# willake/cpu-ray-tracer

Hardware: AMD Instinct MI355X
Metric: Mrays/sec (primary+secondary), 1280x720 64spp path trace — pipelined throughput over 878 consecutive 64-spp windows of one progressive render (single_render = one such render alone) (higher is better)
Workload: dtype f32; 1 GPU; bunny_scene.xml FileScene BVH-SAH path tracer, 1280x720, 64 spp/step (passes=1, depthLimit=5); 1 step = 64 frames = the next spp window of a progressive render; the 878 steps are one crt_render job (14 render kernel launch(es), a wavefront per (tile, 128 consecutive frames), + ordered accumulate), one sync at the end; triangles=4968, parallelism=tile-wave x1

## Files before the change

### cpu-ray-tracer_amd/csrc/abi.cpp

```cpp
#include "../../include/crt_abi.h"
#include "device/launch.h"

#include <cmath>
#include <cstdarg>
#include <cstddef>
#include <cstdio>
#include <cstdlib>
#include <cstring>
#include <deque>
#include <string>
#include <algorithm>
#include <vector>
#include <chrono>

static_assert(sizeof(crt_bvh_node) == 32 && sizeof(crt_tri) == 112 && sizeof(crt_tlas_node) == 32, "reference layouts");
static_assert(sizeof(crt::NodePair) == 64 && sizeof(crt::LeafTri) == 48 && sizeof(crt::ShadeTri) == 64 && sizeof(crt::TlasNode) == 32 &&
              sizeof(crt::Instance) == 128 && sizeof(crt::Material) == 32 && offsetof(crt::Instance, T) == 64, "device layouts");
static_assert(sizeof(crt_counters) == sizeof(crt::Counters), "counter layout");
static_assert(sizeof(crt_kd_node) == 48 && sizeof(crt::KdNode) == sizeof(crt_kd_node) && sizeof(crt::AltTri) == 48, "flat KD node (uploaded as it comes), alternative accelerators' triangle record");
static_assert(offsetof(crt::PrimDev, red) == 536 && sizeof(crt::PrimDev) == 552, "PrimDev: 134 floats, then the two texel pointers");
static_assert(sizeof(crt::BlasAltDesc) == 72, "BLAS descriptor");
static_assert(sizeof(crt_shadow_ray) == 28 && sizeof(crt_ray) == 28 && sizeof(crt_hit) == 28, "query records");
static_assert(sizeof(crt_hit_info) == 48 && offsetof(crt_hit_info, material) == 12 && offsetof(crt_hit_info, N) == 16 && offsetof(crt_hit_info, albedo) == 32 && offsetof(crt_hit_info, v) == 44, "crt_hit_info: three 16-byte pieces");
static_assert(sizeof(crt::Instance) == 128 && offsetof(crt::Instance, triCount) == 112, "Instance record");

namespace {

thread_local std::string g_createError;

bool g_hooks = false;
inline const char* hook(const char* name) { return g_hooks ? getenv(name) : nullptr; }

struct EventPair { hipEvent_t a, b; int mode = -1; bool seen = false; };

}

extern "C" uint32_t crt_debug_query_grid(void)
{
    const char* e = hook("CRT_DEBUG_QUERY_GRID");
    const long k = e ? strtol(e, nullptr, 10) : 0;
    return k > 0 ? (uint32_t)(k > 0x7fffffffL ? 0x7fffffffL : k) : 0u;
}

struct crt_ctx {
    crt_config cfg{};
    std::string err;
    hipStream_t stream = nullptr;
    int tilesX = 0, tilesY = 0;
    uint32_t tileFirst = 0, tileStride = 1, tileCount = 0;
    void* dAccOwned = nullptr; void* dAcc = nullptr;
    std::vector<hipStream_t> streams; uint64_t launchSeq = 0;
    struct Region { size_t off, bytes; hipEvent_t freed; bool held = false; };
    std::deque<Region> inflight;
    char* pool = nullptr; size_t poolBytes = 0, poolHead = 0; bool poolCapped = false;
    hipEvent_t mustWait = nullptr;
    std::vector<hipEvent_t> freeEvents;
    std::vector<hipEvent_t> doneEvents;
    struct Ahead { hipEvent_t end; size_t off; const char* slab; uint64_t epoch; uint32_t sppFirst, nf, passes, used; };
    std::deque<Ahead> ahead;
    uint64_t epoch = 1;
    uint64_t tickEpoch = 0; uint32_t tickNextSpp = 0, tickPasses = 0;
    uint32_t aheadFrames = 0;
    hipStream_t aheadStream = nullptr;
    crt::Scene hScene{};
    crt::Counters* dCounters = nullptr;
    uint32_t* dQueryCursor = nullptr;
    int32_t* dInspectCounts = nullptr; void* dInspectWork = nullptr; size_t inspectCap = 0;
    uint32_t* dPixels = nullptr; float* dTileSums = nullptr;
    unsigned long long* dTileClocks = nullptr;
    std::vector<void*> sceneAllocs;
    float meshLo[3] = {0, 0, 0}, meshHi[3] = {0, 0, 0}; bool orderDirty = true;
    uint32_t* dTileOrder = nullptr;
    uint32_t* hTileOrder[2] = {nullptr, nullptr}; hipEvent_t orderCopied[2] = {nullptr, nullptr}; hipEvent_t orderReady = nullptr; int orderFlip = 0;
    bool haveScene = false;
    struct Flat { int32_t kind = 0; uint64_t leafOff = 0, tlasOff = 0, tlasPairOff = 0, instOff = 0, shadeOff = 0; uint32_t tlasNodeCount = 0, maxHeight = 0;
                  uint32_t objects = 0;
                  std::vector<uint64_t> pairBase, triBase; std::vector<uint32_t> nodesUsed, triCount; std::vector<char> geom;
                  std::vector<float> rootBox; } flat;
    char* hStage[2] = {nullptr, nullptr}; size_t stageBytes[2] = {0, 0}; hipEvent_t stageCopied[2] = {nullptr, nullptr}; int stageFlip = 0;
    hipEvent_t sceneReady = nullptr;
    bool havePrim = false; crt::PrimDev prim{}; uint32_t* dPrimTex = nullptr;
    int renderAccel = 0;
    crt::AltAccelDev alt{}; bool haveKd = false, haveGrid = false; std::vector<void*> altAllocs[2]; crt::AltTri* altTris = nullptr; uint32_t altTriCount = 0;
    crt::TlasAltDev blasAlt[2]{}; bool haveBlas[2] = {false, false}; std::vector<void*> blasAllocs[2];
    bool hasAlt(int kind) const { return (kind == CRT_ACCEL_KDTREE && (haveKd || haveBlas[0])) || (kind == CRT_ACCEL_GRID && (haveGrid || haveBlas[1])); }
    char* dStage = nullptr; size_t stageCap = 0;
    static constexpr int kQuerySlots = 64;
    uint32_t* dQuerySlots = nullptr;
    struct QuerySlot { hipEvent_t done = nullptr; bool pending = false; } qslot[kQuerySlots];
    int qslotNext = 0;
    struct RefitPlan { void* dPlan = nullptr; uint32_t* dLevelOff = nullptr; uint32_t levels = 0, rootCode = 0; bool built = false; };
    std::vector<RefitPlan> refitPlans; std::vector<void*> refitAllocs;
    float* dRefitBack = nullptr; float* hRefitBack = nullptr; hipEvent_t refitFence = nullptr, refitDone = nullptr;
    float* dRootBox = nullptr;
    char* dTlasBuild = nullptr; char* hTlasBack = nullptr; size_t tlasBuildBytes = 0;
    hipEvent_t tlasFence = nullptr, tlasBack = nullptr, tlasDone = nullptr, tlasT0 = nullptr, tlasT1 = nullptr; bool tlasTimed = false;
    hipEvent_t altReady = nullptr;
    static constexpr int kLatStages = 4;
    double tuneMs[kLatStages + 1] = {}; int tuneCount[kLatStages + 1] = {};
    hipEvent_t lastRenderEnd = nullptr;
    int latStage = 0;
    int latBest = 0;
    bool latDone = false;
    bool latConfirming = false; std::vector<int> latQueue;
    bool latWarm = false;
    uint32_t latSlots = 0;
    bool latProbed = false;
    std::vector<uint8_t> latL[kLatStages + 1];
    std::vector<uint32_t> latCost[kLatStages + 1];
    uint32_t* dTileCost = nullptr; uint32_t* hTileCost = nullptr; hipEvent_t costCopied = nullptr; bool costPending = false; int costStage = 0;
    uint32_t* dBlockDesc = nullptr; uint32_t* hBlockDesc = nullptr; uint32_t nBlocks = 0, descCap = 0; hipEvent_t descReady = nullptr;
    uint32_t* dJobCost = nullptr; uint32_t* hJobCost = nullptr; hipEvent_t jobCostCopied = nullptr; bool jobCostPending = false, jobCostValid = false;
    uint32_t recWaves = 0, recResident = 0, recWindows = 0; bool recPool = false;
    double poolWindowTicks = 0;
    std::vector<uint32_t> jobCost;
    std::vector<uint32_t> jobOrder;
    uint32_t* dJobDesc = nullptr; uint32_t* hJobDesc = nullptr; uint32_t jobDescCap = 0, jobBlocks = 0, jobHead = 0; hipEvent_t jobDescReady = nullptr;
    uint32_t planWindows = 0, planFrames = 0; bool planPool = false, planValid = false;
    double jobTrialMs[2] = {0, 0};
    std::vector<hipEvent_t> splitEvents;
    size_t splitSeq = 0; uint32_t splitLaunches = 0;
    uint64_t poolMinWaves = 65000;
    bool usePool = true;
    uint32_t ldsBytes = 0;
    std::vector<EventPair> evPool; size_t evUsedRender = 0, evUsedAcc = 0;
    std::deque<EventPair> evRender, evAcc;
    double foldedRenderMs = 0, foldedAccMs = 0; uint32_t foldedLaunches = 0, poolLaunches = 0;

    int fail(int code, const char* fmt, ...)
    {
        char buf[1024];
        va_list ap; va_start(ap, fmt); vsnprintf(buf, sizeof(buf), fmt, ap); va_end(ap);
        err = buf; return code;
    }
    int hip(hipError_t e, const char* what)
    {
        if (e == hipSuccess) return 0;
        return fail(CRT_ERR_DEVICE, "%s: %s", what, hipGetErrorString(e));
    }
    void freeAlt()
    {
        for (auto& v : altAllocs) { for (void* p : v) (void)hipFree(p); v.clear(); }
        if (altTris) (void)hipFree(altTris);
        altTris = nullptr; altTriCount = 0; haveKd = haveGrid = false; alt = crt::AltAccelDev{}; renderAccel = 0;
        for (int k = 0; k < 2; k++) { for (void* p : blasAllocs[k]) (void)hipFree(p); blasAllocs[k].clear(); haveBlas[k] = false; blasAlt[k] = crt::TlasAltDev{}; }
    }
    void freeScene()
    {
        for (void* p : sceneAllocs) (void)hipFree(p);
        sceneAllocs.clear(); haveScene = false; dRootBox = nullptr;
        for (void* p : refitAllocs) (void)hipFree(p);
        refitAllocs.clear(); refitPlans.clear();
        if (dPrimTex) { (void)hipFree(dPrimTex); dPrimTex = nullptr; }
        havePrim = false;
        freeAlt();
    }
};

#define HIPCK(ctx, call) do { hipError_t e_ = (call); if (e_ != hipSuccess) return (ctx)->hip(e_, #call); } while (0)

namespace {

template <class T>
int upload(crt_ctx* c, const std::vector<T>& v, const T** out)
{
    *out = nullptr;
    if (v.empty()) return 0;
    void* d = nullptr;
    HIPCK(c, hipMalloc(&d, v.size() * sizeof(T)));
    c->sceneAllocs.push_back(d);
    HIPCK(c, hipMemcpyAsync(d, v.data(), v.size() * sizeof(T), hipMemcpyHostToDevice, c->stream));
    HIPCK(c, hipStreamSynchronize(c->stream));
    *out = reinterpret_cast<const T*>(d);
    return 0;
}

template <class T>
int upload_array(crt_ctx* c, std::vector<void*>& allocs, const void* src, size_t bytes, const T** out)
{
    *out = nullptr; if (!bytes) return 0;
    void* d = nullptr; HIPCK(c, hipMalloc(&d, bytes)); allocs.push_back(d);
    HIPCK(c, hipMemcpy(d, src, bytes, hipMemcpyHostToDevice)); *out = static_cast<const T*>(d); return 0;
}

int bvh_height(crt_ctx* c, const crt_bvh& b, uint32_t* heightOut)
{
    std::vector<std::pair<uint32_t, uint32_t>> st; st.push_back({0u, 0u});
    uint32_t h = 0; size_t visited = 0;
    while (!st.empty()) {
        auto [n, d] = st.back(); st.pop_back();
        if (++visited > (size_t)b.nodesUsed) return c->fail(CRT_ERR_INVALID, "BVH node graph is not a tree");
        const crt_bvh_node& nd = b.nodes[n];
        if (nd.triCount > 0) { if (d > h) h = d; continue; }
        if (nd.leftFirst == 0 || nd.leftFirst + 1 >= b.nodesUsed) return c->fail(CRT_ERR_INVALID, "BVH child index out of range (node %u)", n);
        st.push_back({nd.leftFirst, d + 1}); st.push_back({nd.leftFirst + 1, d + 1});
    }
    *heightOut = h;
    return 0;
}

int wait_queries(crt_ctx* c)
{
    for (auto& q : c->qslot) if (q.pending) { HIPCK(c, hipEventSynchronize(q.done)); q.pending = false; }
    return 0;
}

int order_behind_queries(crt_ctx* c)
{
    for (auto& q : c->qslot) {
        if (!q.pending) continue;
        const hipError_t e = hipEventQuery(q.done);
        if (e == hipSuccess) { q.pending = false; continue; }
        if (e != hipErrorNotReady) return c->hip(e, "hipEventQuery(query)");
        HIPCK(c, hipStreamWaitEvent(c->stream, q.done, 0));
    }
    return 0;
}

int drain_all(crt_ctx* c)
{
    for (auto st : c->streams) HIPCK(c, hipStreamSynchronize(st));
    if (c->aheadStream) HIPCK(c, hipStreamSynchronize(c->aheadStream));
    HIPCK(c, hipStreamSynchronize(c->stream));
    return wait_queries(c);
}

}

extern "C" {

int crt_abi_version(void) { return CRT_ABI_VERSION; }

void crt_debug_enable_hooks(int on) { g_hooks = on != 0; }

int crt_device_count(void)
{
    int n = 0;
    if (hipGetDeviceCount(&n) != hipSuccess) return 0;
    return n;
}

const char* crt_last_error(crt_ctx* ctx) { return ctx ? ctx->err.c_str() : g_createError.c_str(); }

int crt_create(crt_ctx** out, const crt_config* cfg)
{
    if (!out || !cfg) { g_createError = "crt_create: null argument"; return CRT_ERR_INVALID; }
    *out = nullptr;
    setenv("GPU_MAX_HW_QUEUES", "16", 0);
    if (cfg->width < 16 || cfg->height < 16) { g_createError = "crt_create: width and height must be at least one 16x16 tile"; return CRT_ERR_INVALID; }
    int ndev = 0;
    hipError_t e = hipGetDeviceCount(&ndev);
    if (e != hipSuccess || ndev == 0) {
        g_createError = "crt_create: no HIP device visible (this library has no CPU path)";
        return CRT_ERR_NO_DEVICE;
    }
    if (cfg->device < 0 || cfg->device >= ndev) { g_createError = "crt_create: device ordinal out of range"; return CRT_ERR_INVALID; }
    crt_ctx* c = new crt_ctx();
    c->cfg = *cfg;
    if (const char* k = hook("CRT_RENDER_KERNEL")) {
        c->usePool = strcmp(k, "tiles") != 0;
        if (!strcmp(k, "pool_always")) c->poolMinWaves = 0;
    }
    if (c->cfg.depthLimit < 0) c->cfg.depthLimit = 5;
    if (c->cfg.depthLimit > 5) { g_createError = "crt_create: depthLimit > 5 unsupported (throughput stack holds 5 factors; reference default is 5)"; delete c; return CRT_ERR_UNSUPPORTED; }
    if (c->cfg.maxFramesPerLaunch <= 0) c->cfg.maxFramesPerLaunch = c->cfg.collectStats ? 64 : 4096;
    if (c->cfg.maxFramesPerLaunch > 64) c->cfg.maxFramesPerLaunch = c->cfg.maxFramesPerLaunch / 64 * 64;
    if (c->cfg.renderStreams < 0) c->cfg.renderStreams = 0;
    c->tilesX = cfg->width / 16; c->tilesY = cfg->height / 16;
    const int tiles = c->tilesX * c->tilesY;
    int first = cfg->tileFirst, stride = cfg->tileStride <= 0 ? 1 : cfg->tileStride, count = cfg->tileCount;
    if (count < 0) { first = 0; stride = 1; count = tiles; }
    if (first < 0 || (count > 0 && (long long)first + (long long)(count - 1) * stride >= tiles)) {
        g_createError = "crt_create: tile range exceeds the image"; delete c; return CRT_ERR_INVALID;
    }
    c->tileFirst = (uint32_t)first; c->tileStride = (uint32_t)stride; c->tileCount = (uint32_t)count;

    auto bail = [&](hipError_t he, const char* what) {
        g_createError = std::string("crt_create: ") + what + ": " + hipGetErrorString(he);
        crt_destroy(c); return CRT_ERR_DEVICE;
    };
    if ((e = hipSetDevice(cfg->device)) != hipSuccess) return bail(e, "hipSetDevice");
    if ((e = hipStreamCreateWithFlags(&c->stream, hipStreamNonBlocking)) != hipSuccess) return bail(e, "hipStreamCreate");
    const size_t px = (size_t)cfg->width * cfg->height;
    if ((e = hipMalloc(&c->dAccOwned, px * 16)) != hipSuccess) return bail(e, "hipMalloc(accumulator)");
    c->dAcc = c->dAccOwned;
    if ((e = hipMemsetAsync(c->dAcc, 0, px * 16, c->stream)) != hipSuccess) return bail(e, "hipMemset(accumulator)");
    if ((e = hipMalloc((void**)&c->dPixels, px * 4)) != hipSuccess) return bail(e, "hipMalloc(pixels)");
    if ((e = hipMemsetAsync(c->dPixels, 0, px * 4, c->stream)) != hipSuccess) return bail(e, "hipMemset(pixels)");
    if ((e = hipMalloc((void**)&c->dTileSums, (size_t)tiles * 4)) != hipSuccess) return bail(e, "hipMalloc(tileSums)");
    if ((e = hipMemsetAsync(c->dTileSums, 0, (size_t)tiles * 4, c->stream)) != hipSuccess) return bail(e, "hipMemset(tileSums)");
    if ((e = hipMalloc((void**)&c->dCounters, sizeof(crt::Counters))) != hipSuccess) return bail(e, "hipMalloc(counters)");
    if ((e = hipMemsetAsync(c->dCounters, 0, sizeof(crt::Counters), c->stream)) != hipSuccess) return bail(e, "hipMemset(counters)");
    if ((e = hipMalloc((void**)&c->dQueryCursor, 64)) != hipSuccess) return bail(e, "hipMalloc(query cursor)");
    if ((e = hipMalloc((void**)&c->dQuerySlots, crt_ctx::kQuerySlots * 64)) != hipSuccess) return bail(e, "hipMalloc(query cursor slots)");
    if (c->cfg.collectStats && count > 0) {
        if ((e = hipMalloc((void**)&c->dTileClocks, (size_t)count * 144)) != hipSuccess) return bail(e, "hipMalloc(tileClocks)");
        if ((e = hipMemsetAsync(c->dTileClocks, 0, (size_t)count * 144, c->stream)) != hipSuccess) return bail(e, "hipMemset(tileClocks)");
    }
    memset(&c->hScene, 0, sizeof(c->hScene));
    const float aspect = (float)cfg->width / (float)cfg->height;
    crt::Scene& s = c->hScene;
    s.camPos[0] = 0; s.camPos[1] = 0; s.camPos[2] = -2;
    s.topLeft[0] = -aspect; s.topLeft[1] = 1; s.topLeft[2] = 0;
    s.topRight[0] = aspect; s.topRight[1] = 1; s.topRight[2] = 0;
    s.bottomLeft[0] = -aspect; s.bottomLeft[1] = -1; s.bottomLeft[2] = 0;
    s.W = cfg->width; s.H = cfg->height; s.invW = 1.0f / cfg->width; s.invH = 1.0f / cfg->height;
    s.depthLimit = c->cfg.depthLimit;
    if ((e = hipStreamSynchronize(c->stream)) != hipSuccess) return bail(e, "hipStreamSynchronize");
    *out = c;
    return CRT_OK;
}

void crt_destroy(crt_ctx* c)
{
    if (!c) return;
    (void)hipSetDevice(c->cfg.device);
    for (auto st : c->streams) (void)hipStreamSynchronize(st);
    if (c->aheadStream) (void)hipStreamSynchronize(c->aheadStream);
    if (c->stream) (void)hipStreamSynchronize(c->stream);
    for (auto& q : c->qslot) if (q.done) { if (q.pending) (void)hipEventSynchronize(q.done); (void)hipEventDestroy(q.done); }
    if (c->dQuerySlots) (void)hipFree(c->dQuerySlots);
    if (c->altReady) (void)hipEventDestroy(c->altReady);
    if (c->refitFence) (void)hipEventDestroy(c->refitFence);
    if (c->refitDone) (void)hipEventDestroy(c->refitDone);
    if (c->dRefitBack) (void)hipFree(c->dRefitBack);
    if (c->hRefitBack) (void)hipHostFree(c->hRefitBack);
    for (hipEvent_t e : {c->tlasFence, c->tlasBack, c->tlasDone, c->tlasT0, c->tlasT1}) if (e) (void)hipEventDestroy(e);
    if (c->dTlasBuild) (void)hipFree(c->dTlasBuild);
    if (c->hTlasBack) (void)hipHostFree(c->hTlasBack);
    c->freeScene();
    for (auto& a : c->ahead) (void)hipEventDestroy(a.end);
    if (c->aheadStream) (void)hipStreamDestroy(c->aheadStream);
    for (auto& ev : c->evPool) { (void)hipEventDestroy(ev.a); (void)hipEventDestroy(ev.b); }
    for (auto& ev : c->evRender) { (void)hipEventDestroy(ev.a); (void)hipEventDestroy(ev.b); }
    for (auto& ev : c->evAcc) { (void)hipEventDestroy(ev.a); (void)hipEventDestroy(ev.b); }
    if (c->dAccOwned) (void)hipFree(c->dAccOwned);
    for (auto st : c->streams) { (void)hipStreamSynchronize(st); (void)hipStreamDestroy(st); }
    for (auto& r : c->inflight) (void)hipEventDestroy(r.freed);
    for (auto e : c->freeEvents) (void)hipEventDestroy(e);
    if (c->mustWait) (void)hipEventDestroy(c->mustWait);
    if (c->pool) (void)hipFree(c->pool);
    for (auto e : c->doneEvents) (void)hipEventDestroy(e);
    if (c->dPixels) (void)hipFree(c->dPixels);
    if (c->dTileSums) (void)hipFree(c->dTileSums);
    if (c->dCounters) (void)hipFree(c->dCounters);
    if (c->dQueryCursor) (void)hipFree(c->dQueryCursor);
    if (c->dInspectCounts) (void)hipFree(c->dInspectCounts);
    if (c->dInspectWork) (void)hipFree(c->dInspectWork);
    if (c->dTileClocks) (void)hipFree(c->dTileClocks);
    if (c->dTileOrder) (void)hipFree(c->dTileOrder);
    if (c->dTileCost) (void)hipFree(c->dTileCost);
    if (c->dJobCost) (void)hipFree(c->dJobCost);
    if (c->dJobDesc) (void)hipFree(c->dJobDesc);
    if (c->hJobDesc) (void)hipHostFree(c->hJobDesc);
    if (c->jobDescReady) (void)hipEventDestroy(c->jobDescReady);
    if (c->hJobCost) (void)hipHostFree(c->hJobCost);
    if (c->jobCostCopied) (void)hipEventDestroy(c->jobCostCopied);
    for (auto e : c->splitEvents) (void)hipEventDestroy(e);
    if (c->hTileCost) (void)hipHostFree(c->hTileCost);
    if (c->costCopied) (void)hipEventDestroy(c->costCopied);
    if (c->dBlockDesc) (void)hipFree(c->dBlockDesc);
    if (c->hBlockDesc) (void)hipHostFree(c->hBlockDesc);
    if (c->descReady) (void)hipEventDestroy(c->descReady);
    if (c->dStage) (void)hipFree(c->dStage);
    for (int k = 0; k < 2; k++) { if (c->hTileOrder[k]) (void)hipHostFree(c->hTileOrder[k]); if (c->orderCopied[k]) (void)hipEventDestroy(c->orderCopied[k]); }
    for (int k = 0; k < 2; k++) { if (c->hStage[k]) (void)hipHostFree(c->hStage[k]); if (c->stageCopied[k]) (void)hipEventDestroy(c->stageCopied[k]); }
    if (c->stream) (void)hipStreamDestroy(c->stream);
    delete c;
}

int crt_upload_scene(crt_ctx* c, const crt_scene_desc* sd)
{
    if (!c || !sd) return CRT_ERR_INVALID;
    c->epoch++;
    HIPCK(c, hipSetDevice(c->cfg.device));
    if (sd->kind != CRT_SCENE_FILE && sd->kind != CRT_SCENE_TLAS) return c->fail(CRT_ERR_INVALID, "unknown scene kind %d", sd->kind);
    if (!sd->bvhs || sd->bvhCount == 0) return c->fail(CRT_ERR_INVALID, "scene has no acceleration structure");
    if (sd->kind == CRT_SCENE_FILE && sd->bvhCount != 1) return c->fail(CRT_ERR_INVALID, "CRT_SCENE_FILE takes exactly one BVH (FileScene::acc)");
    if (sd->kind == CRT_SCENE_TLAS && (sd->bvhCount > 256 || !sd->tlasNodes || sd->tlasNodeCount < 2 * sd->bvhCount))
        return c->fail(CRT_ERR_INVALID, "TLAS scene needs <= 256 BLAS (tlas_bvh.cpp:21) and 2*blasCount TLAS nodes");
    if (sd->textureCount == 0 || !sd->textures) return c->fail(CRT_ERR_INVALID, "floor and skydome textures are required");
    if (sd->floorTexture < 0 || sd->floorTexture >= (int)sd->textureCount || sd->skyTexture < 0 || sd->skyTexture >= (int)sd->textureCount)
        return c->fail(CRT_ERR_INVALID, "floor/sky texture index out of range");
    for (uint32_t i = 0; i < sd->textureCount; i++)
        if (!sd->textures[i].pixels || sd->textures[i].width <= 0 || sd->textures[i].height <= 0) return c->fail(CRT_ERR_INVALID, "texture %u is empty", i);
    if (sd->materialCount > 0 && !sd->materials) return c->fail(CRT_ERR_INVALID, "materialCount is %u but materials is NULL", sd->materialCount);
    for (uint32_t i = 0; i < sd->materialCount; i++)
        if (sd->materials[i].texture >= (int)sd->textureCount) return c->fail(CRT_ERR_INVALID, "material %u: texture index out of range", i);
    if (sd->kind == CRT_SCENE_FILE) {
        if (!sd->objMatIdx || sd->objCount == 0) return c->fail(CRT_ERR_INVALID, "CRT_SCENE_FILE needs objMatIdx");
        for (uint32_t i = 0; i < sd->objCount; i++)
            if (sd->objMatIdx[i] < 0 || sd->objMatIdx[i] >= (int)sd->materialCount) return c->fail(CRT_ERR_INVALID, "objMatIdx entry out of range");
    }

    uint64_t nPairs = 0, nTris = 0;
    uint32_t maxHeight = 0;
    for (uint32_t bi = 0; bi < sd->bvhCount; bi++) {
        const crt_bvh& b = sd->bvhs[bi];
        if (!b.nodes || !b.triangles || !b.triangleIndices || b.nodesUsed == 0 || b.triCount == 0) return c->fail(CRT_ERR_INVALID, "BVH %u is empty", bi);
        if ((b.nodesUsed & 1u) == 0) return c->fail(CRT_ERR_INVALID, "BVH %u: nodesUsed must be odd (root + child pairs)", bi);
        if (sd->kind == CRT_SCENE_TLAS && (b.matIdx < 0 || b.matIdx >= (int)sd->materialCount)) return c->fail(CRT_ERR_INVALID, "BLAS %u: matIdx out of range", bi);
        if (sd->kind == CRT_SCENE_TLAS && b.objIdx != (int)bi + 2)
            return c->fail(CRT_ERR_INVALID, "BLAS %u: objIdx must be %u (TLASFileScene numbers objects from 2, tlas_file_scene.cpp:13,51-53)", bi, bi + 2);
        uint32_t h = 0; int r = bvh_height(c, b, &h); if (r) return r;
        if (h > maxHeight) maxHeight = h;
        nPairs += b.nodesUsed / 2; nTris += b.triCount;
    }
    const uint64_t pairBytes = nPairs ? nPairs * 64 : 64;
    const uint64_t leafOffB = pairBytes, leafBytes = (nTris + 1) * 48;
    const uint64_t tlasOffB = (leafOffB + leafBytes + 63) & ~63ull;
    const uint64_t tlasBytes = (sd->kind == CRT_SCENE_TLAS) ? (uint64_t)sd->tlasNodeCount * 32 : 0;
    const uint64_t tlasPairOffB = (tlasOffB + tlasBytes + 63) & ~63ull;
    const uint64_t tlasPairBytes = (sd->kind == CRT_SCENE_TLAS) ? (uint64_t)sd->tlasNodeCount * 32 : 0;
    const uint64_t instOffB = (tlasPairOffB + tlasPairBytes + 127) & ~127ull;
    const uint64_t instBytes = (sd->kind == CRT_SCENE_TLAS) ? (uint64_t)sd->bvhCount * 128 : 0;
    const uint64_t shadeOffB = (instOffB + instBytes + 63) & ~63ull;
    const uint64_t total = shadeOffB + nTris * 64;
    if (total >= crt::kMaxGeomBytes) return c->fail(CRT_ERR_UNSUPPORTED, "scene geometry needs %llu bytes; this build addresses 4 GiB", (unsigned long long)total);
    if (sd->kind == CRT_SCENE_TLAS && sd->tlasNodeCount > 0x7fffu) return c->fail(CRT_ERR_UNSUPPORTED, "TLAS node index exceeds 15 bits");

    std::vector<char> geom((size_t)total, 0);
    crt::NodePair* pairs = reinterpret_cast<crt::NodePair*>(geom.data());
// ... 475 lines not shown
    for (uint32_t i = 0; i < n; i++) if (lanes[i] == 0 || lanes[i] > 64 || (64 % lanes[i]) != 0) return CRT_ERR_INVALID;
    std::vector<uint8_t> L; const double t = solve_block_table(std::vector<uint8_t>(lanes, lanes + n), std::vector<uint32_t>(cost, cost + n), budget, L);
    if (n) memcpy(out, L.data(), n);
    if (T) *T = t;
    return CRT_OK;
}
static double lat_budget(crt_ctx* c)
{
    if (!c->latSlots) c->latSlots = crt_render_resident_waves(c->cfg.device, c->hScene.kind, c->ldsBytes);
    double share = 0.98;
    if (const char* e = hook("CRT_LAT_BUDGET")) { const double v = atof(e); if (v > 0) share = v; }
    return share * (double)c->latSlots;
}

static int upload_block_table(crt_ctx* c, const std::vector<uint8_t>& lanes, const std::vector<uint32_t>& cost)
{
    const uint32_t n = c->tileCount;
    std::vector<uint32_t> order(n);
    for (uint32_t i = 0; i < n; i++) order[i] = i;
    std::stable_sort(order.begin(), order.end(), [&](uint32_t a, uint32_t b) { return cost[a] > cost[b]; });
    std::vector<uint32_t> table; table.reserve((size_t)n * 2);
    for (uint32_t r = 0; r < n; r++) {
        const uint32_t tl = order[r], L = lanes[tl];
        for (uint32_t base = 0; base < 64u; base += L) table.push_back(block_desc(tl, base, L, 0u));
    }
    if (table.size() > 0x7fffffffull) return c->fail(CRT_ERR_INVALID, "block table too large");
    if (hook("CRT_LAT_VERBOSE")) fprintf(stderr, "[crt] latency table: %zu wavefronts for %u tiles (slowest tile of the base stage %.2f ms)\n", table.size(), n, n ? cost[order[0]] * 1e-5 : 0.0);
    if (c->descCap < table.size()) {
        if (c->dBlockDesc) (void)hipFree(c->dBlockDesc);
        if (c->hBlockDesc) (void)hipHostFree(c->hBlockDesc);
        c->dBlockDesc = nullptr; c->hBlockDesc = nullptr; c->descCap = 0;
        const size_t cap = table.size() + table.size() / 2;
        HIPCK(c, hipMalloc((void**)&c->dBlockDesc, cap * 4));
        HIPCK(c, hipHostMalloc((void**)&c->hBlockDesc, cap * 4, hipHostMallocDefault));
        c->descCap = (uint32_t)cap;
    } else if (c->descReady) HIPCK(c, hipEventSynchronize(c->descReady));
    if (!c->descReady) HIPCK(c, hipEventCreateWithFlags(&c->descReady, hipEventDisableTiming));
    memcpy(c->hBlockDesc, table.data(), table.size() * 4);
    { const int r = order_behind_ahead(c); if (r) return r; }
    HIPCK(c, hipMemcpyAsync(c->dBlockDesc, c->hBlockDesc, table.size() * 4, hipMemcpyHostToDevice, c->stream));
    HIPCK(c, hipEventRecord(c->descReady, c->stream));
    c->nBlocks = (uint32_t)table.size();
    return 0;
}

static int next_block_table(crt_ctx* c)
{
    const uint32_t n = c->tileCount; const int K = crt_ctx::kLatStages;
    const int s = c->costStage;
    if (s == 0 && !c->latWarm && !c->latProbed) { c->latWarm = true; return 0; }
    c->latCost[s].assign(c->hTileCost, c->hTileCost + n);
    if (s == 0 && !c->latProbed) c->latL[0].assign(n, 64);
    if (c->tuneCount[s] && (c->latBest == s || !c->tuneCount[c->latBest] || c->tuneMs[s] < c->tuneMs[c->latBest])) c->latBest = s;
    bool last = s >= K;
    std::vector<std::pair<double, uint32_t>> steps;
    if (const char* e = hook("CRT_LAT_POLICY")) {
        for (const char* p = e; *p;) {
            char* q = nullptr; const double sh = strtod(p, &q); if (q == p || *q != ':') break;
            const long L = strtol(q + 1, &q, 10); if (L < 1 || L > 64 || (64 % L) != 0) break;
            steps.push_back({sh, (uint32_t)L});
            p = (*q == ',') ? q + 1 : q; if (*q != ',') break;
        }
        if (s >= 1) last = true;
    }
    auto install = [&](int stage) -> int {
        if ((stage != 0 || c->latProbed) && stage != c->latStage) { const int r = upload_block_table(c, c->latL[stage], c->latCost[stage]); if (r) return r; }
        c->latStage = stage; return 0;
    };
    auto fastest = [&](int except) { int b = -1; for (int k = 0; k <= K; k++) if (k != except && c->tuneCount[k] && (b < 0 || c->tuneMs[k] < c->tuneMs[b])) b = k; return b; };
    auto finish = [&]() -> int {
        c->latDone = true; c->latConfirming = false;
        const int b = fastest(-1); c->latBest = b < 0 ? 0 : b;
        if (hook("CRT_LAT_FORCE")) c->latBest = s;
        if (hook("CRT_LAT_VERBOSE")) { fprintf(stderr, "[crt] latency stages:"); for (int k = 0; k <= K; k++) if (c->tuneCount[k]) fprintf(stderr, " %d: %.2f ms", k, c->tuneMs[k]); fprintf(stderr, " -> %d\n", c->latBest); }
        return install(c->latBest);
    };
    if (c->latConfirming) {
        if (!c->latQueue.empty()) c->latQueue.erase(c->latQueue.begin());
        if (!c->latQueue.empty()) return install(c->latQueue.front());
        return finish();
    }
    if (last) {
        const int a = fastest(-1), b2 = fastest(a);
        if (hook("CRT_LAT_FORCE") || a < 0 || b2 < 0) return finish();
        c->latQueue = {a, b2}; c->latConfirming = true;
        return install(a);
    }
    const int b = c->latBest;
    const std::vector<uint8_t>& baseL = c->latL[b]; const std::vector<uint32_t>& baseC = c->latCost[b];
    uint32_t top = 0; for (uint32_t i = 0; i < n; i++) top = baseC[i] > top ? baseC[i] : top;
    std::vector<uint8_t>& L = c->latL[s + 1]; L = baseL;
    if (!steps.empty()) {
        for (uint32_t i = 0; i < n; i++)
            for (const auto& st : steps) if (top > 0 && (double)baseC[i] >= st.first * (double)top) { L[i] = (uint8_t)st.second; break; }
    } else {
        const double T = solve_block_table(c->latL[s], c->latCost[s], lat_budget(c), L);
        if (hook("CRT_LAT_VERBOSE")) fprintf(stderr, "[crt] stage %d: aim %.2f ms\n", s + 1, T * 1e-5);
    }
    const int r = upload_block_table(c, L, steps.empty() ? c->latCost[s] : baseC);
    if (r) return r;
    c->latStage = s + 1;
    return 0;
}

static void harvest_tuning(crt_ctx* c)
{
    for (auto& ev : c->evRender) {
        if (ev.mode < 0 || ev.seen) continue;
        if (hipEventQuery(ev.b) != hipSuccess) break;
        float t = 0;
        if (hipEventElapsedTime(&t, ev.a, ev.b) == hipSuccess) {
            if (ev.mode >= 100) { double& m = c->jobTrialMs[ev.mode - 100]; m = (m > 0 && m < t) ? m : t; }
            else { c->tuneMs[ev.mode] = c->tuneCount[ev.mode] ? (c->tuneMs[ev.mode] < t ? c->tuneMs[ev.mode] : t) : t; c->tuneCount[ev.mode]++; }
        }
        ev.seen = true;
    }
}

static void fold_completed(crt_ctx* c, std::deque<EventPair>& list, double* ms, uint32_t* count)
{
    while (list.size() > 64 && hipEventQuery(list.front().b) == hipSuccess) {
        float t = 0;
        if (hipEventElapsedTime(&t, list.front().a, list.front().b) == hipSuccess) *ms += t;
        if (count) (*count)++;
        c->evPool.push_back(list.front()); list.pop_front();
    }
}

static int take_event(crt_ctx* c, std::deque<EventPair>& list, EventPair* out)
{
    EventPair ev;
    if (c->evPool.empty()) {
        HIPCK(c, hipEventCreate(&ev.a)); HIPCK(c, hipEventCreate(&ev.b));
    } else { ev = c->evPool.back(); c->evPool.pop_back(); }
    ev.mode = -1; ev.seen = false;
    list.push_back(ev); *out = ev;
    return 0;
}

static int release_ahead_region(crt_ctx* c, const crt_ctx::Ahead& a)
{
    for (auto& r : c->inflight)
        if (r.held && r.off == a.off) { HIPCK(c, hipEventRecord(r.freed, c->stream)); r.held = false; return 0; }
    return c->fail(CRT_ERR_DEVICE, "render-ahead region at %zu is not in the slab ring", a.off);
}

static int discard_ahead(crt_ctx* c)
{
    while (!c->ahead.empty()) {
        const crt_ctx::Ahead a = c->ahead.front(); c->ahead.pop_front();
        HIPCK(c, hipStreamWaitEvent(c->stream, a.end, 0));
        c->doneEvents.push_back(a.end);
        const int r = release_ahead_region(c, a); if (r) return r;
    }
    c->aheadFrames = 0;
    return 0;
}

static int ensure_pool(crt_ctx* c, uint32_t frames, uint32_t passes, uint32_t* maxFOut)
{
    const size_t windowBytes = window_bytes(c, passes);
    uint32_t maxF = (uint32_t)c->cfg.maxFramesPerLaunch;
    uint32_t maxW = maxF >= 64u ? maxF / 64u : 1u;
    const uint32_t wantW = (frames + 63u) / 64u;
    const uint32_t callW = wantW < maxW ? wantW : maxW;
    size_t want = (size_t)callW * windowBytes * (wantW > callW ? 2u : 1u);
    if (want < 8 * windowBytes) want = 8 * windowBytes;
    if (want > c->poolBytes && !(c->poolCapped && windowBytes <= c->poolBytes)) {
        { const int r = discard_ahead(c); if (r) return r; }
        HIPCK(c, hipStreamSynchronize(c->stream));
        for (auto st : c->streams) HIPCK(c, hipStreamSynchronize(st));
        if (c->aheadStream) HIPCK(c, hipStreamSynchronize(c->aheadStream));
        for (auto& r : c->inflight) c->freeEvents.push_back(r.freed);
        c->inflight.clear(); c->poolHead = 0;
        if (c->pool) { HIPCK(c, hipFree(c->pool)); c->pool = nullptr; c->poolBytes = 0; }
        size_t freeB = 0, totalB = 0;
        HIPCK(c, hipMemGetInfo(&freeB, &totalB));
        const size_t budget = freeB / 2;
        if (budget < windowBytes) return c->fail(CRT_ERR_DEVICE, "not enough free HBM for one 64-frame sample slab (%zu bytes needed, %zu free)", windowBytes, freeB);
        c->poolCapped = want > budget;
        if (want > budget) want = budget;
        want = want / windowBytes * windowBytes;
        HIPCK(c, hipMalloc((void**)&c->pool, want));
        c->poolBytes = want;
    }
    {
        uint32_t fitW = (uint32_t)(c->poolBytes / windowBytes);
        if (wantW > fitW && fitW >= 2) fitW /= 2;
        if (maxW > fitW) maxW = fitW;
    }
    if (maxF >= 64u) maxF = maxW * 64u;
    *maxFOut = maxF;
    return 0;
}

int crt_reserve(crt_ctx* c, uint32_t frames, uint32_t passes)
{
    if (!c) return CRT_ERR_INVALID;
    if (passes < 1 || passes > 4) return c->fail(CRT_ERR_INVALID, "passes must be 1..4");
    HIPCK(c, hipSetDevice(c->cfg.device));
    { const int r = discard_ahead(c); if (r) return r; }
    if (c->tileCount == 0 || frames == 0) return CRT_OK;
    uint32_t maxF = 0;
    return ensure_pool(c, frames, passes, &maxF);
}

static int take_region(crt_ctx* c, size_t need, hipStream_t st, size_t* offOut)
{
    for (;;) {
        bool ok = false; size_t off = 0;
        if (c->inflight.empty()) { off = 0; ok = need <= c->poolBytes; }
        else {
            const size_t tail = c->inflight.front().off;
            if (c->poolHead > tail) {
                if (c->poolBytes - c->poolHead >= need) { off = c->poolHead; ok = true; }
                else if (tail >= need) { off = 0; ok = true; }
            } else if (c->poolHead < tail && tail - c->poolHead >= need) { off = c->poolHead; ok = true; }
        }
        if (ok) {
            if (c->mustWait) HIPCK(c, hipStreamWaitEvent(st, c->mustWait, 0));
            c->poolHead = off + need; *offOut = off;
            return 0;
        }
        if (c->inflight.empty()) return c->fail(CRT_ERR_DEVICE, "slab pool of %zu bytes cannot hold a launch of %zu bytes", c->poolBytes, need);
        if (c->inflight.front().held) return 1;
        if (c->mustWait) c->freeEvents.push_back(c->mustWait);
        c->mustWait = c->inflight.front().freed;
        c->inflight.pop_front();
    }
}

static size_t job_cost_clk_offset(const crt_ctx* c) { return (((size_t)c->tileCount + 1u) & ~(size_t)1u) * 4u; }
static size_t job_cost_bytes(const crt_ctx* c) { return job_cost_clk_offset(c) + 24u; }

static int adopt_job_costs(crt_ctx* c)
{
    const uint32_t n = c->tileCount;
    c->jobCost.assign(c->hJobCost, c->hJobCost + n);
    {
        const unsigned long long* clk = reinterpret_cast<const unsigned long long*>(reinterpret_cast<const char*>(c->hJobCost) + job_cost_clk_offset(c));
        const double s0 = (clk[0] && clk[1] && clk[1] > ~clk[0]) ? (double)(clk[1] - ~clk[0]) : 0.0;
        const double drain = (double)clk[2] / (double)(c->recResident ? c->recResident : 1u);
        c->poolWindowTicks = 0;
        if (c->recWindows && (double)c->recWaves >= 1.5 * (double)c->recResident && s0 > 0) c->poolWindowTicks = (s0 + drain) / (double)c->recWindows / (c->recPool ? 1.0 : 1.2);
        if (hook("CRT_LAT_VERBOSE")) fprintf(stderr, "[crt] measured %u windows with %s: %u wavefronts, last one started %.2f ms after the first, then %.2f ms of drain -> %.3f ms of machine time per window under the pool\n", c->recWindows, c->recPool ? "the pool" : "one stream per lane", c->recWaves, s0 * 1e-5, drain * 1e-5, c->poolWindowTicks * 1e-5);
    }
    c->jobOrder.resize(n);
    for (uint32_t i = 0; i < n; i++) c->jobOrder[i] = i;
    std::stable_sort(c->jobOrder.begin(), c->jobOrder.end(), [&](uint32_t a, uint32_t b) { return c->jobCost[a] > c->jobCost[b]; });
    c->jobCostValid = true; c->planValid = false;
    return upload_tile_order(c, c->jobOrder);
}

static void plan_job(const crt_ctx* c, uint32_t windows, uint32_t frames, bool pool, std::vector<uint32_t>& table, uint32_t* head)
{
    table.clear(); *head = 0;
    const uint32_t n = c->tileCount;
    if (!c->jobCostValid || windows < 2u || windows > 64u || n > 0x10000u || c->cfg.collectStats || hook("CRT_SPLIT_OFF")) return;
    if (pool && c->streams.size() < 2) return;
    if (const char* e = hook("CRT_SPLIT_FORCE")) {
        const uint32_t h = std::min<uint32_t>((uint32_t)atoi(e), pool ? n - 1u : n);
        static const uint32_t Ls[4] = {64u, 16u, 2u, 1u};
        for (uint32_t r = 0; r < (pool ? h : n); r++) { const uint32_t L = r < h ? Ls[r & 3u] : 64u; for (uint32_t w = 0; w < windows; w++) for (uint32_t b0 = 0; b0 < 64u; b0 += L) table.push_back(block_desc(c->jobOrder[r], b0, L, w)); }
        *head = h; return;
    }
    double poolLong = 2.4, wideLoad = 1.1, poolSlots = 4096.0, wideMt = 1.2, narrowSlots = 3500.0;
    if (const char* e = hook("CRT_PLAN_NARROW_SLOTS")) narrowSlots = atof(e);
    const double K = (double)windows;
    double costSum = 0; for (uint32_t v : c->jobCost) costSum += (double)v;
    const double perCost = (c->poolWindowTicks > 0 && costSum > 0) ? c->poolWindowTicks / costSum : 1.0 / poolSlots;
    auto cheapest = [&](double v, double T, int* cls) -> double {
        if (pool && poolLong * v <= T) { *cls = 0; return K * v * perCost; }
        if (wideLoad * v <= T) { *cls = 1; return K * wideMt * v * perCost; }
        int k = 1; while (k < 6 && kLatG[k] * v > T) k++;
        *cls = 2 + k; return K * (64.0 / kLatLanes[k]) * kLatG[k] * v / narrowSlots;
    };
    auto machine = [&](double T) { double m = 0; int cls; for (uint32_t v : c->jobCost) m += cheapest((double)v, T, &cls); return m; };
    const double top = (double)c->jobCost[c->jobOrder[0]];
    double lo = top * kLatG[6], hi = std::max(poolLong * top, machine(1e30)) * 1.01;
    if (machine(lo) <= lo) hi = lo;
    else for (int it = 0; it < 50; it++) { const double mid = 0.5 * (lo + hi); if (machine(mid) <= mid) hi = mid; else lo = mid; }
    const double T = hi;
    uint32_t h = 0, narrow = 0; std::vector<uint8_t> lanes(n, 64);
    for (uint32_t r = 0; r < n; r++) {
        int cls; (void)cheapest((double)c->jobCost[c->jobOrder[r]], T, &cls);
        if (cls != 0) h = r + 1u;
        if (cls >= 2) { lanes[r] = (uint8_t)kLatLanes[cls - 2]; narrow++; }
    }
    if (pool && h >= n) h = n - 1u;
    if (hook("CRT_LAT_VERBOSE")) fprintf(stderr, "[crt] job of %u windows, %u tiles: makespan aim %.1f ms (most expensive tile %.2f ms); %u tiles to the block table, %u of them narrow, %s\n", windows, n, T * 1e-5, top * 1e-5, pool ? h : (narrow ? n : 0u), narrow, pool ? "rest to the pool" : "no pool");
    if (pool ? h == 0u : narrow == 0u) return;
    const uint32_t upto = pool ? h : n;
    for (uint32_t r = 0; r < upto; r++) {
        const uint32_t L = lanes[r];
        for (uint32_t w = 0; w < windows; w++) {
            const uint32_t fw = std::min(64u, frames - w * 64u);
            for (uint32_t b0 = 0; b0 < fw; b0 += L) table.push_back(block_desc(c->jobOrder[r], b0, L, w));
        }
    }
    if (table.size() > (4u << 20)) { table.clear(); *head = 0; return; }
    *head = pool ? h : 0u;
}

static int install_job_plan(crt_ctx* c, uint32_t windows, uint32_t frames, bool pool)
{
    if (c->planValid && c->planWindows == windows && c->planFrames == frames && c->planPool == pool) return 0;
    std::vector<uint32_t> table; uint32_t head = 0;
    plan_job(c, windows, frames, pool, table, &head);
    c->planValid = true; c->planWindows = windows; c->planFrames = frames; c->planPool = pool; c->jobHead = head; c->jobBlocks = (uint32_t)table.size();
    c->jobTrialMs[0] = c->jobTrialMs[1] = 0;
    if (table.empty()) return 0;
    if (c->jobDescCap < table.size()) {
        if (c->dJobDesc) (void)hipFree(c->dJobDesc);
        if (c->hJobDesc) (void)hipHostFree(c->hJobDesc);
        c->dJobDesc = nullptr; c->hJobDesc = nullptr; c->jobDescCap = 0;
        const size_t cap = table.size() + table.size() / 2;
        HIPCK(c, hipMalloc((void**)&c->dJobDesc, cap * 4));
        HIPCK(c, hipHostMalloc((void**)&c->hJobDesc, cap * 4, hipHostMallocDefault));
        c->jobDescCap = (uint32_t)cap;
    } else if (c->jobDescReady) HIPCK(c, hipEventSynchronize(c->jobDescReady));
    if (!c->jobDescReady) HIPCK(c, hipEventCreateWithFlags(&c->jobDescReady, hipEventDisableTiming));
    memcpy(c->hJobDesc, table.data(), table.size() * 4);
    { const int r = order_behind_ahead(c); if (r) return r; }
    HIPCK(c, hipMemcpyAsync(c->dJobDesc, c->hJobDesc, table.size() * 4, hipMemcpyHostToDevice, c->stream));
    HIPCK(c, hipEventRecord(c->jobDescReady, c->stream));
    return 0;
}

struct Launch {
    hipStream_t st = nullptr; EventPair ev{}; void* slab = nullptr; uint32_t sppFirst = 0, nf = 0, passes = 1, windows = 1;
    const uint32_t* blockDesc = nullptr; uint32_t nBlocks = 0;
    bool wantCost = false, wantJobCost = false, pool = false;
    uint32_t head = 0, jobBlocks = 0; unsigned long long* jobClk = nullptr;
};

static int next_block_table(crt_ctx* c);
static int probe_tile_costs(crt_ctx* c, hipStream_t st);

static int tuner_prepare(crt_ctx* c, Launch& L)
{
    int r;
    const bool gpuIdle = !c->lastRenderEnd || hipEventQuery(c->lastRenderEnd) == hipSuccess;
    if (L.nf <= 64u && L.nf >= 8u && gpuIdle && !c->cfg.collectStats && c->tileCount <= 0x10000u && !hook("CRT_LAT_OFF")) {
        if (c->costPending && hipEventQuery(c->costCopied) == hipSuccess) { c->costPending = false; harvest_tuning(c); if ((r = next_block_table(c))) return r; }
        if (c->latStage == 0 && !c->latProbed && !c->latWarm && !c->costPending && L.nf == 64u && !hook("CRT_LAT_POLICY") && !hook("CRT_LAT_NO_PROBE")) { if ((r = probe_tile_costs(c, L.st))) return r; }
        const int stage = c->latStage;
        if (stage || c->latProbed) { L.blockDesc = c->dBlockDesc; L.nBlocks = c->nBlocks; HIPCK(c, hipStreamWaitEvent(L.st, c->descReady, 0)); }
        L.wantCost = (!c->latDone && !c->costPending) || (c->latDone && hook("CRT_LAT_RECORD"));
        c->evRender.back().mode = c->latDone ? -1 : stage;
        if (L.wantCost && !c->latDone) c->costStage = stage;
    }
    if (L.wantCost) {
        if (!c->dTileCost) {
            HIPCK(c, hipMalloc((void**)&c->dTileCost, (size_t)c->tileCount * 4));
            HIPCK(c, hipHostMalloc((void**)&c->hTileCost, (size_t)c->tileCount * 4, hipHostMallocDefault));
            HIPCK(c, hipEventCreateWithFlags(&c->costCopied, hipEventDisableTiming));
        }
        else HIPCK(c, hipStreamWaitEvent(L.st, c->costCopied, 0));
        HIPCK(c, hipMemsetAsync(c->dTileCost, 0, (size_t)c->tileCount * 4, L.st));
    }
    return 0;
}

static int planner_prepare(crt_ctx* c, Launch& L)
{
    int r;
    if (L.nf > 64u && !c->cfg.collectStats) {
        if (c->jobCostPending && hipEventQuery(c->jobCostCopied) == hipSuccess) { c->jobCostPending = false; if ((r = adopt_job_costs(c))) return r; HIPCK(c, hipStreamWaitEvent(L.st, c->orderReady, 0)); }
        L.wantJobCost = !c->jobCostValid && !c->jobCostPending && L.nf >= 128u;
        if (L.wantJobCost) {
            if (!c->dJobCost) {
                HIPCK(c, hipMalloc((void**)&c->dJobCost, job_cost_bytes(c)));
                HIPCK(c, hipHostMalloc((void**)&c->hJobCost, job_cost_bytes(c), hipHostMallocDefault));
                HIPCK(c, hipEventCreateWithFlags(&c->jobCostCopied, hipEventDisableTiming));
            } else HIPCK(c, hipStreamWaitEvent(L.st, c->jobCostCopied, 0));
            HIPCK(c, hipMemsetAsync(c->dJobCost, 0, job_cost_bytes(c), L.st));
        }
    }
    const uint64_t minWaves = c->poolMinWaves != 65000u ? c->poolMinWaves : (c->jobCostValid ? 43000u : 65000u);
    L.pool = c->usePool && c->hScene.ref16ok && (uint64_t)c->tileCount * L.windows >= minWaves && (c->poolMinWaves == 0 || L.nf > 64u);
    if (L.nf > 64u && c->jobCostValid) {
        if ((r = install_job_plan(c, L.windows, L.nf, L.pool))) return r;
        int use = 1;
        if (c->jobBlocks && !hook("CRT_PLAN_NO_TRIAL")) {
            if (c->jobTrialMs[1] > 0 && c->jobTrialMs[0] > 0) use = c->jobTrialMs[1] <= c->jobTrialMs[0] ? 1 : 0;
            else if (c->jobTrialMs[1] > 0 && c->jobTrialMs[0] == 0) use = 0;
            c->evRender.back().mode = 100 + use;
        }
        if (use) { L.head = c->jobHead; L.jobBlocks = c->jobBlocks; }
    }
    if (L.jobBlocks) HIPCK(c, hipStreamWaitEvent(L.st, c->jobDescReady, 0));
    if (L.wantJobCost) {
        L.jobClk = reinterpret_cast<unsigned long long*>(reinterpret_cast<char*>(c->dJobCost) + job_cost_clk_offset(c));
        c->recPool = L.pool; c->recWindows = L.windows;
        c->recWaves = L.pool ? c->tileCount * ((L.nf + crt_pool_streams(L.nf) - 1u) / crt_pool_streams(L.nf)) : c->tileCount * L.windows;
        c->recResident = L.pool ? 4096u : 5120u;
    }
    return 0;
}

static hipError_t launch_render_kernels(crt_ctx* c, const Launch& L)
{
    hipStream_t st = L.st;
    hipError_t le = hipSuccess;
    auto join = [&](hipStream_t other) -> hipError_t {
        if (other == st) return hipSuccess;
        hipError_t e = hipSuccess;
        if (c->splitEvents.size() < 32) { hipEvent_t ne; e = hipEventCreateWithFlags(&ne, hipEventDisableTiming); if (e == hipSuccess) c->splitEvents.push_back(ne); }
        if (e == hipSuccess) { hipEvent_t je = c->splitEvents[c->splitSeq++ % c->splitEvents.size()]; e = hipEventRecord(je, other); if (e == hipSuccess) e = hipStreamWaitEvent(st, je, 0); }
        return e;
    };
    auto launch_table = [&](const uint32_t* desc, uint32_t nBlocks, uint32_t* cost) -> hipError_t {
        return crt_launch_render(&c->hScene, L.slab, c->dCounters, c->dTileClocks, c->dTileOrder, c->tileFirst, c->tileStride, c->tileCount, (uint32_t)c->tilesX,
                                 L.sppFirst, L.nf, L.passes, c->ldsBytes, 0, desc, nBlocks, cost, 0u, nullptr, st);
    };
    if (L.pool) {
        void* scratch = (char*)L.slab + (size_t)L.windows * sample_bytes_per_window(c, L.passes);
        hipStream_t st2 = st;
        if (L.jobBlocks) {
            le = launch_table(c->dJobDesc, L.jobBlocks, nullptr);
            st2 = c->streams[(size_t)(c->launchSeq++ % c->streams.size())];
            if (le == hipSuccess && st2 != st) le = hipStreamWaitEvent(st2, L.ev.a, 0);
        }
        if (le == hipSuccess)
            le = crt_launch_render_pool(&c->hScene, L.slab, scratch, c->dCounters, c->dTileClocks, c->dTileOrder, c->tileFirst, c->tileStride, c->tileCount, (uint32_t)c->tilesX,
                                        L.sppFirst, L.nf, L.passes, c->cfg.collectStats, L.jobBlocks ? L.head : 0u, L.wantJobCost ? c->dJobCost : nullptr, L.jobClk, st2);
        if (L.jobBlocks && le == hipSuccess) le = join(st2);
    } else if (L.jobBlocks) {
        le = launch_table(c->dJobDesc, L.jobBlocks, nullptr);
    } else if (L.blockDesc && L.nBlocks) {
        le = launch_table(L.blockDesc, L.nBlocks, L.wantCost ? c->dTileCost : nullptr);
    } else {
        le = crt_launch_render(&c->hScene, L.slab, c->dCounters, c->dTileClocks, c->dTileOrder, c->tileFirst, c->tileStride, c->tileCount, (uint32_t)c->tilesX,
                               L.sppFirst, L.nf, L.passes, c->ldsBytes, c->cfg.collectStats, nullptr, 0u,
                               L.wantCost ? c->dTileCost : (L.wantJobCost ? c->dJobCost : nullptr), 0u, L.jobClk, st);
    }
    if (L.jobBlocks && le == hipSuccess) c->splitLaunches++;
    return le;
}

static int probe_tile_costs(crt_ctx* c, hipStream_t st)
{
    const uint32_t n = c->tileCount;
    if (!c->dTileCost) {
        HIPCK(c, hipMalloc((void**)&c->dTileCost, (size_t)n * 4));
        HIPCK(c, hipHostMalloc((void**)&c->hTileCost, (size_t)n * 4, hipHostMallocDefault));
        HIPCK(c, hipEventCreateWithFlags(&c->costCopied, hipEventDisableTiming));
    } else HIPCK(c, hipEventSynchronize(c->costCopied));
    const auto tp0 = std::chrono::steady_clock::now();
    HIPCK(c, crt_launch_probe(&c->hScene, c->tileFirst, c->tileStride, n, (uint32_t)c->tilesX, c->dTileCost, st));
    HIPCK(c, hipMemcpyAsync(c->hTileCost, c->dTileCost, (size_t)n * 4, hipMemcpyDeviceToHost, st));
    HIPCK(c, hipEventRecord(c->costCopied, st));
    HIPCK(c, hipStreamSynchronize(st));
    const auto tp1 = std::chrono::steady_clock::now();
    std::vector<uint32_t>& est = c->latCost[0]; est.assign(c->hTileCost, c->hTileCost + n);
    for (uint32_t i = 0; i < n; i++) est[i] += 18u * crt_probe_paths();
    std::vector<uint8_t>& L = c->latL[0]; L.assign(n, 64);
    solve_block_table(std::vector<uint8_t>(n, 64), est, lat_budget(c), L);
    c->latProbed = true;
    bool any = false; for (uint32_t i = 0; i < n; i++) any = any || L[i] != 64;
    if (!any) { c->latProbed = false; return 0; }
    const auto tp2 = std::chrono::steady_clock::now();
    const int r = upload_block_table(c, L, est);
    if (hook("CRT_LAT_VERBOSE")) { const auto tp3 = std::chrono::steady_clock::now(); auto ms = [](auto a, auto b) { return std::chrono::duration<double, std::milli>(b - a).count(); };
        fprintf(stderr, "[crt] cost probe: launch + wait %.3f ms, table solved in %.3f ms, uploaded in %.3f ms\n", ms(tp0, tp1), ms(tp1, tp2), ms(tp2, tp3)); }
    return r;
}

static int launch_frames(crt_ctx* c, uint32_t sppFirst, uint32_t nf, uint32_t passes, hipStream_t st, crt_ctx::Ahead* ahead)
{
    const size_t windowBytes = window_bytes(c, passes);
    size_t off = 0; int r;
    if ((r = take_region(c, (size_t)((nf + 63u) / 64u) * windowBytes, st, &off))) return r;
    if (c->orderReady) HIPCK(c, hipStreamWaitEvent(st, c->orderReady, 0));
    if (c->sceneReady) HIPCK(c, hipStreamWaitEvent(st, c->sceneReady, 0));
    void* slab = c->pool + off;
    EventPair ev;
    harvest_tuning(c);
    fold_completed(c, c->evRender, &c->foldedRenderMs, &c->foldedLaunches); fold_completed(c, c->evAcc, &c->foldedAccMs, nullptr);
    if ((r = take_event(c, c->evRender, &ev))) return r;
    struct PairGuard { crt_ctx* c; bool armed; ~PairGuard() { if (armed && !c->evRender.empty()) { c->evPool.push_back(c->evRender.back()); c->evRender.pop_back(); } } } pairGuard{c, true};
    Launch L; L.st = st; L.ev = ev; L.slab = slab; L.sppFirst = sppFirst; L.nf = nf; L.passes = passes; L.windows = (nf + 63u) / 64u;
    if ((r = tuner_prepare(c, L))) return r;
    if ((r = planner_prepare(c, L))) return r;
    HIPCK(c, hipEventRecord(ev.a, st));
    const bool pool = L.pool, wantCost = L.wantCost, wantJobCost = L.wantJobCost;
    const hipError_t le = hook("CRT_DEBUG_FAIL_LAUNCH") ? hipErrorInvalidConfiguration  : launch_render_kernels(c, L);
    if (le != hipSuccess) {
        return c->hip(le, pool ? "launch of render_pool_kernel" : "launch of render_tiles_kernel");
    }
    if (pool) c->poolLaunches++;
    HIPCK(c, hipEventRecord(ev.b, st));
    pairGuard.armed = false;
    c->lastRenderEnd = ev.b;
    if (wantJobCost) {
        HIPCK(c, hipMemcpyAsync(c->hJobCost, c->dJobCost, job_cost_bytes(c), hipMemcpyDeviceToHost, st));
        HIPCK(c, hipEventRecord(c->jobCostCopied, st));
        c->jobCostPending = true;
    }
    if (wantCost && !pool && !c->latDone) {
        HIPCK(c, hipMemcpyAsync(c->hTileCost, c->dTileCost, (size_t)c->tileCount * 4, hipMemcpyDeviceToHost, st));
        HIPCK(c, hipEventRecord(c->costCopied, st));
        c->costPending = true;
    }
    crt_ctx::Region reg; reg.off = off; reg.bytes = (size_t)((nf + 63u) / 64u) * windowBytes;
    if (c->freeEvents.empty()) HIPCK(c, hipEventCreateWithFlags(&reg.freed, hipEventDisableTiming));
    else { reg.freed = c->freeEvents.back(); c->freeEvents.pop_back(); }
    if (ahead) {
        hipEvent_t end = nullptr;
        if (c->doneEvents.empty()) { const hipError_t e = hipEventCreateWithFlags(&end, hipEventDisableTiming); if (e != hipSuccess) { c->freeEvents.push_back(reg.freed); return c->hip(e, "hipEventCreate"); } }
        else { end = c->doneEvents.back(); c->doneEvents.pop_back(); }
        const hipError_t e = hipEventRecord(end, st);
        if (e != hipSuccess) { c->doneEvents.push_back(end); c->freeEvents.push_back(reg.freed); return c->hip(e, "hipEventRecord"); }
        reg.held = true;
        c->inflight.push_back(reg);
        *ahead = crt_ctx::Ahead{end, off, (const char*)slab, c->epoch, sppFirst, nf, passes, 0u};
        return 0;
    }
    HIPCK(c, hipStreamWaitEvent(c->stream, ev.b, 0));
    if ((r = take_event(c, c->evAcc, &ev))) return r;
    HIPCK(c, hipEventRecord(ev.a, c->stream));
    HIPCK(c, crt_launch_accumulate(slab, c->dAcc, c->tileFirst, c->tileStride, c->tileCount, (uint32_t)c->tilesX, (uint32_t)c->cfg.width, nf, passes, c->stream));
    HIPCK(c, hipEventRecord(ev.b, c->stream));
    HIPCK(c, hipEventRecord(reg.freed, c->stream));
    c->inflight.push_back(reg);
    return 0;
}

int crt_render(crt_ctx* c, uint32_t spp_first, uint32_t frames, uint32_t passes)
{
    if (!c) return CRT_ERR_INVALID;
    if (!c->haveScene && !c->havePrim) return c->fail(CRT_ERR_STATE, "crt_render before crt_upload_scene");
    if (passes < 1 || passes > 4) return c->fail(CRT_ERR_INVALID, "passes must be 1..4 (the reference's UI range, renderer.cpp:178)");
    HIPCK(c, hipSetDevice(c->cfg.device));
    { int r = discard_ahead(c); if (r) return r; }
    if (c->tileCount == 0 || frames == 0) return CRT_OK;
    { int r = update_tile_order(c); if (r) return r; }
    if (c->streams.empty()) {
        int n = c->cfg.renderStreams;
        if (n <= 0) n = 7;
        if (n > 16) n = 16;
        if (c->cfg.collectStats) n = 1;
        c->streams.resize((size_t)n);
        for (auto& st : c->streams) HIPCK(c, hipStreamCreateWithFlags(&st, hipStreamNonBlocking));
    }
    uint32_t maxF = 0;
    { int r = ensure_pool(c, frames, passes, &maxF); if (r) return r; }
    const size_t windowBytes = window_bytes(c, passes);
    if (c->renderAccel != 0 || c->havePrim) {
        for (uint32_t f0 = 0; f0 < frames; f0 += maxF) {
            const uint32_t nf = (frames - f0 < maxF) ? frames - f0 : maxF;
            size_t off = 0; int r;
            if ((r = take_region(c, (size_t)((nf + 63u) / 64u) * windowBytes, c->stream, &off))) return r;
            if (c->sceneReady) HIPCK(c, hipStreamWaitEvent(c->stream, c->sceneReady, 0));
            void* slab = c->pool + off;
            if (c->havePrim) HIPCK(c, crt_launch_render_prim(&c->hScene, &c->prim, slab, c->dCounters, c->tileFirst, c->tileStride, c->tileCount, (uint32_t)c->tilesX, spp_first + f0 * passes, nf, passes, c->stream));
            else HIPCK(c, crt_launch_render_alt(c->renderAccel, &c->hScene, &c->alt, &c->blasAlt[c->renderAccel - 1], slab, c->dCounters, c->tileFirst, c->tileStride, c->tileCount, (uint32_t)c->tilesX, spp_first + f0 * passes, nf, passes, c->stream));
            HIPCK(c, crt_launch_accumulate(slab, c->dAcc, c->tileFirst, c->tileStride, c->tileCount, (uint32_t)c->tilesX, (uint32_t)c->cfg.width, nf, passes, c->stream));
            crt_ctx::Region reg; reg.off = off; reg.bytes = (size_t)((nf + 63u) / 64u) * windowBytes;
            if (c->freeEvents.empty()) HIPCK(c, hipEventCreateWithFlags(&reg.freed, hipEventDisableTiming));
            else { reg.freed = c->freeEvents.back(); c->freeEvents.pop_back(); }
            HIPCK(c, hipEventRecord(reg.freed, c->stream));
            c->inflight.push_back(reg);
        }
        return CRT_OK;
    }
    for (uint32_t f0 = 0; f0 < frames; f0 += maxF) {
        const uint32_t nf = (frames - f0 < maxF) ? frames - f0 : maxF;
        const int r = launch_frames(c, spp_first + f0 * passes, nf, passes, c->streams[(size_t)(c->launchSeq++ % c->streams.size())], nullptr);
        if (r) return r > 0 ? c->fail(CRT_ERR_DEVICE, "slab ring blocked by a render-ahead region") : r;
    }
    return CRT_OK;
}

int crt_sync(crt_ctx* c)
{
    if (!c) return CRT_ERR_INVALID;
    HIPCK(c, hipSetDevice(c->cfg.device));
    HIPCK(c, hipStreamSynchronize(c->stream));
    for (auto st : c->streams) HIPCK(c, hipStreamSynchronize(st));
    if (c->aheadStream) HIPCK(c, hipStreamSynchronize(c->aheadStream));
    return CRT_OK;
}

int crt_clear(crt_ctx* c)
{
    if (!c) return CRT_ERR_INVALID;
    HIPCK(c, hipSetDevice(c->cfg.device));
    HIPCK(c, hipMemsetAsync(c->dAcc, 0, (size_t)c->cfg.width * c->cfg.height * 16, c->stream));
    return CRT_OK;
}

int crt_read_accumulator(crt_ctx* c, float* host)
{
    if (!c || !host) return CRT_ERR_INVALID;
    HIPCK(c, hipSetDevice(c->cfg.device));
    HIPCK(c, hipMemcpyAsync(host, c->dAcc, (size_t)c->cfg.width * c->cfg.height * 16, hipMemcpyDeviceToHost, c->stream));
    HIPCK(c, hipStreamSynchronize(c->stream));
    return CRT_OK;
}

static int read_screen(crt_ctx* c, uint32_t* hostPixels, float* energy)
{
    const int tiles = c->tilesX * c->tilesY;
    if (hostPixels) HIPCK(c, hipMemcpyAsync(hostPixels, c->dPixels, (size_t)c->cfg.width * c->cfg.height * 4, hipMemcpyDeviceToHost, c->stream));
    std::vector<float> sums(tiles);
    HIPCK(c, hipMemcpyAsync(sums.data(), c->dTileSums, (size_t)tiles * 4, hipMemcpyDeviceToHost, c->stream));
    HIPCK(c, hipStreamSynchronize(c->stream));
    if (energy) { float e = 0; for (int i = 0; i < tiles; i++) e += sums[i]; *energy = e; }
    return CRT_OK;
}

int crt_resolve_screen(crt_ctx* c, float scale, uint32_t* hostPixels, float* energy)
{
    if (!c) return CRT_ERR_INVALID;
    HIPCK(c, hipSetDevice(c->cfg.device));
    HIPCK(c, crt_launch_resolve(c->dAcc, c->dPixels, c->dTileSums, c->tileFirst, c->tileStride, c->tileCount, (uint32_t)c->tilesX, (uint32_t)c->cfg.width, scale, c->stream));
    return read_screen(c, hostPixels, energy);
}

static constexpr uint32_t kAheadMaxFrames = 256;

static int launch_ahead(crt_ctx* c, uint32_t sppFirst, uint32_t passes)
{
    if (!c->aheadStream) {
        int least = 0, greatest = 0;
        HIPCK(c, hipDeviceGetStreamPriorityRange(&least, &greatest));
        HIPCK(c, hipStreamCreateWithPriority(&c->aheadStream, hipStreamNonBlocking, least));
    }
    uint32_t nf = c->aheadFrames ? std::min(2u * c->aheadFrames, kAheadMaxFrames) : 64u;
    if (nf > (uint32_t)c->cfg.maxFramesPerLaunch) nf = (uint32_t)c->cfg.maxFramesPerLaunch;
    const uint32_t poolW = (uint32_t)(c->poolBytes / window_bytes(c, passes));
    if (nf > poolW / 2u * 64u) nf = poolW / 2u * 64u;
    if (nf == 0 || c->streams.empty()) return 0;
    hipStream_t st = hook("CRT_AHEAD_NORMAL_PRIORITY") ? c->streams[(size_t)(c->launchSeq++ % c->streams.size())] : c->aheadStream;
    crt_ctx::Ahead a{};
    const int r = launch_frames(c, sppFirst, nf, passes, st, &a);
    if (r < 0) return r;
    if (r > 0) return 0;
    c->ahead.push_back(a); c->aheadFrames = nf;
    return 0;
}

int crt_tick(crt_ctx* c, uint32_t spp, uint32_t passes, uint32_t* hostPixels, float* hostRgba, float* energy)
{
    if (!c) return CRT_ERR_INVALID;
    if (!c->haveScene && !c->havePrim) return c->fail(CRT_ERR_STATE, "crt_tick before crt_upload_scene");
    if (passes < 1 || passes > 4) return c->fail(CRT_ERR_INVALID, "passes must be 1..4 (the reference's UI range, renderer.cpp:178)");
    HIPCK(c, hipSetDevice(c->cfg.device));
    const float scale = 1.0f / (float)(spp + passes);
    const bool eligible = !c->cfg.collectStats && c->renderAccel == 0 && !c->havePrim && c->tileCount > 0;
    const bool streak = eligible && c->tickEpoch == c->epoch && spp == c->tickNextSpp && passes == c->tickPasses;
    c->tickEpoch = c->epoch; c->tickNextSpp = spp + passes; c->tickPasses = passes;
    const bool hit = !c->ahead.empty() && c->ahead.front().epoch == c->epoch && c->ahead.front().passes == passes &&
                     spp == c->ahead.front().sppFirst + c->ahead.front().used * passes;
    int r;
    if (hit) {
        crt_ctx::Ahead& a = c->ahead.front();
        const uint32_t f = a.used++;
        HIPCK(c, hipStreamWaitEvent(c->stream, a.end, 0));
        HIPCK(c, crt_launch_commit_frame(a.slab + (size_t)(f / 64u) * sample_bytes_per_window(c, passes), f % 64u, passes, c->dAcc, c->dPixels, c->dTileSums,
                                         c->tileFirst, c->tileStride, c->tileCount, (uint32_t)c->tilesX, (uint32_t)c->cfg.width, scale, c->stream));
        if (a.used == a.nf) {
            const crt_ctx::Ahead done = a; c->ahead.pop_front();
            c->doneEvents.push_back(done.end);
            if ((r = release_ahead_region(c, done))) return r;
        }
        if (c->ahead.size() < 2u) {
            const uint32_t next = c->ahead.empty() ? spp + passes : c->ahead.back().sppFirst + c->ahead.back().nf * passes;
            if ((r = launch_ahead(c, next, passes))) return r;
        }
    } else {
        if ((r = crt_render(c, spp, 1, passes))) return r;
        HIPCK(c, crt_launch_resolve(c->dAcc, c->dPixels, c->dTileSums, c->tileFirst, c->tileStride, c->tileCount, (uint32_t)c->tilesX, (uint32_t)c->cfg.width, scale, c->stream));
    }
    if (hostRgba) HIPCK(c, hipMemcpyAsync(hostRgba, c->dAcc, (size_t)c->cfg.width * c->cfg.height * 16, hipMemcpyDeviceToHost, c->stream));
    if ((r = read_screen(c, hostPixels, energy))) return r;
    if (!hit && streak && (r = launch_ahead(c, spp + passes, passes))) return r;
    return CRT_OK;
}

int crt_whitted_tick(crt_ctx* c, uint32_t* hostPixels)
{
    if (!c) return CRT_ERR_INVALID;
    if (!c->haveScene) return c->fail(CRT_ERR_STATE, "crt_whitted_tick before crt_upload_scene");
    HIPCK(c, hipSetDevice(c->cfg.device));
    HIPCK(c, crt_launch_whitted(&c->hScene, c->renderAccel, &c->alt, c->renderAccel ? &c->blasAlt[c->renderAccel - 1] : nullptr, c->dAcc, c->dPixels, c->dCounters, c->ldsBytes, c->stream));
    if (hostPixels) HIPCK(c, hipMemcpyAsync(hostPixels, c->dPixels, (size_t)c->cfg.width * c->cfg.height * 4, hipMemcpyDeviceToHost, c->stream));
    HIPCK(c, hipStreamSynchronize(c->stream));
    return CRT_OK;
}

int crt_whitted_tick_inspect(crt_ctx* c, int inspect, int32_t peakTraversalIn, int32_t peakTestsIn, uint32_t* hostPixels, int32_t* hostTraversed, int32_t* hostTested, crt_whitted_metrics* metrics)
{
    if (!c) return CRT_ERR_INVALID;
    if (inspect < CRT_INSPECT_NONE || inspect > CRT_INSPECT_TESTS) return c->fail(CRT_ERR_INVALID, "crt_whitted_tick_inspect: inspect must be CRT_INSPECT_NONE, _TRAVERSAL or _TESTS");
    if (peakTraversalIn < 0 || peakTestsIn < 0) return c->fail(CRT_ERR_INVALID, "crt_whitted_tick_inspect: a peak cannot be negative");
    if (!c->haveScene) return c->fail(CRT_ERR_STATE, "crt_whitted_tick_inspect before crt_upload_scene");
    HIPCK(c, hipSetDevice(c->cfg.device));
    const size_t n = (size_t)c->cfg.width * c->cfg.height;
    if (n > c->inspectCap) {
        HIPCK(c, hipStreamSynchronize(c->stream));
        if (c->dInspectCounts) (void)hipFree(c->dInspectCounts);
        if (c->dInspectWork) (void)hipFree(c->dInspectWork);
        c->dInspectCounts = nullptr; c->dInspectWork = nullptr; c->inspectCap = 0;
        HIPCK(c, hipMalloc((void**)&c->dInspectCounts, n * 2 * sizeof(int32_t)));
        HIPCK(c, hipMalloc(&c->dInspectWork, crt_whitted_inspect_work_bytes((uint32_t)n)));
        c->inspectCap = n;
    }
    int32_t* dTrav = c->dInspectCounts; int32_t* dTested = c->dInspectCounts + n;
    HIPCK(c, crt_launch_whitted_inspect(&c->hScene, c->renderAccel, &c->alt, c->renderAccel ? &c->blasAlt[c->renderAccel - 1] : nullptr, inspect,
                                        inspect == CRT_INSPECT_TESTS ? peakTestsIn : peakTraversalIn, c->dAcc, c->dPixels, c->dCounters, dTrav, dTested, c->dInspectWork, c->ldsBytes, c->stream));
    static_assert(sizeof(crt_whitted_metrics) == 32, "crt::InspectSums (kernels.hip) is read back into this record");
    crt_whitted_metrics m;
    if (hostPixels) HIPCK(c, hipMemcpyAsync(hostPixels, c->dPixels, n * 4, hipMemcpyDeviceToHost, c->stream));
    if (hostTraversed) HIPCK(c, hipMemcpyAsync(hostTraversed, dTrav, n * 4, hipMemcpyDeviceToHost, c->stream));
    if (hostTested) HIPCK(c, hipMemcpyAsync(hostTested, dTested, n * 4, hipMemcpyDeviceToHost, c->stream));
    if (metrics) HIPCK(c, hipMemcpyAsync(&m, c->dInspectWork, sizeof(m), hipMemcpyDeviceToHost, c->stream));
    HIPCK(c, hipStreamSynchronize(c->stream));
    if (metrics) {
        if (m.peakTraversal < peakTraversalIn) m.peakTraversal = peakTraversalIn;
        if (m.peakTests < peakTestsIn) m.peakTests = peakTestsIn;
        *metrics = m;
    }
    return CRT_OK;
}

static int stage(crt_ctx* c, size_t bytes)
{
// ... 484 lines not shown
        HIPCK(c, hipStreamWaitEvent(st, c->tlasFence, 0));
    }
    HIPCK(c, hipMemcpyAsync(const_cast<char*>(c->hScene.geom) + f.tlasOff, c->dTlasBuild + sizeof(crt::TlasBuildHeader), imageBytes, hipMemcpyDeviceToDevice, st));
    HIPCK(c, hipEventRecord(c->tlasDone, st));
    c->sceneReady = c->tlasDone;
    if (st != c->stream) HIPCK(c, hipStreamWaitEvent(c->stream, c->tlasDone, 0));
    c->epoch++;
    memcpy(f.geom.data() + f.tlasOff, image, imageBytes);
    const crt::TlasNode* nodes = reinterpret_cast<const crt::TlasNode*>(image);
    adopt_tlas(c, h.height, nodes[0].lo, nodes[0].hi);
    if (tlasOut)
        for (uint32_t i = 0; i < 2u * N; i++) {
            const crt::TlasNode& n = nodes[i]; crt_tlas_node& o = tlasOut[i];
            memcpy(o.aabbMin, n.lo, 12); memcpy(o.aabbMax, n.hi, 12);
            const bool leaf = (n.ref & 0xC0000000u) == crt::kRefTlasLeaf;
            o.leftRight = leaf ? 0u : ((n.ref & 0x7fffu) | (((n.ref >> 15) & 0x7fffu) << 16));
            o.BLAS = leaf ? (n.ref & 0xffffu) : 0u;
        }
    return CRT_OK;
}

extern "C" int crt_internal_read_device(crt_ctx* c, void* dst, const void* d_src, size_t bytes, void* stream)
{
    if (!c || !dst) return CRT_ERR_INVALID;
    HIPCK(c, hipSetDevice(c->cfg.device));
    int r; hipStream_t st = nullptr;
    if ((r = check_device_buffer(c, d_src, bytes, "crt_internal_read_device")) || (r = caller_stream(c, stream, "crt_internal_read_device", &st))) return r;
    HIPCK(c, hipMemcpyAsync(dst, d_src, bytes, hipMemcpyDeviceToHost, st));
    HIPCK(c, hipStreamSynchronize(st));
    return CRT_OK;
}

extern "C" int crt_debug_tlas_build_ms(crt_ctx* c, float* ms)
{
    if (!c || !ms) return CRT_ERR_INVALID;
    if (!c->tlasTimed) return c->fail(CRT_ERR_STATE, "crt_debug_tlas_build_ms: no timed crt_update_transforms_device (debug hooks off?)");
    HIPCK(c, hipEventSynchronize(c->tlasT1));
    HIPCK(c, hipEventElapsedTime(ms, c->tlasT0, c->tlasT1));
    return CRT_OK;
}

int crt_is_occluded(crt_ctx* c, int accel, const crt_shadow_ray* rays, int32_t* occluded, size_t n)
{
    if (!c) return CRT_ERR_INVALID;
    int r;
    if ((r = query_check(c, accel, true, n, "crt_is_occluded"))) return r;
    if (n == 0) return CRT_OK;
    if (!rays || !occluded) return c->fail(CRT_ERR_INVALID, "crt_is_occluded: NULL buffer");
    return query_host(c, true, accel, rays, occluded, n);
}

static int shade_check(crt_ctx* c, bool hitInfo, size_t n, const char* what)
{
    if (hitInfo && c->havePrim) return c->fail(CRT_ERR_UNSUPPORTED, "%s: GetHitInfo of the PrimitiveScene is not served (crt_abi.h)", what);
    return query_check(c, 0, false, n, what);
}

static uint32_t file_tri_count(const crt_ctx* c) { return c->flat.kind == CRT_SCENE_FILE ? c->flat.triCount[0] : 0u; }

int crt_get_hit_info(crt_ctx* c, const crt_ray* rays, const crt_hit* hits, crt_hit_info* out, size_t n)
{
    if (!c) return CRT_ERR_INVALID;
    int r;
    if ((r = shade_check(c, true, n, "crt_get_hit_info"))) return r;
    if (n == 0) return CRT_OK;
    if (!rays || !hits || !out) return c->fail(CRT_ERR_INVALID, "crt_get_hit_info: NULL buffer");
    const crt_ctx::Flat& f = c->flat;
    for (size_t i = 0; i < n; i++)
        if (!crt::hit_record_ok(hits[i].objIdx, hits[i].triIdx, f.objects, [&](uint32_t k) { return f.triCount[f.kind == CRT_SCENE_TLAS ? k : 0]; }))
            return c->fail(CRT_ERR_INVALID, "crt_get_hit_info: record %zu names objIdx %d, triIdx %d; the scene has objects -1 .. %u and that object's BVH fewer triangles", i, hits[i].objIdx, hits[i].triIdx, f.objects + 1);
    HIPCK(c, hipSetDevice(c->cfg.device));
    if ((r = stage(c, n * (sizeof(crt_hit_info) + sizeof(crt_ray) + sizeof(crt_hit))))) return r;
    char* dOut = c->dStage; char* dRays = dOut + n * sizeof(crt_hit_info); char* dHits = dRays + n * sizeof(crt_ray);
    HIPCK(c, hipMemcpyAsync(dRays, rays, n * sizeof(crt_ray), hipMemcpyHostToDevice, c->stream));
    HIPCK(c, hipMemcpyAsync(dHits, hits, n * sizeof(crt_hit), hipMemcpyHostToDevice, c->stream));
    HIPCK(c, crt_launch_hit_info(&c->hScene, dRays, dHits, dOut, (uint32_t)n, f.objects, file_tri_count(c), c->stream));
    HIPCK(c, hipMemcpyAsync(out, dOut, n * sizeof(crt_hit_info), hipMemcpyDeviceToHost, c->stream));
    HIPCK(c, hipStreamSynchronize(c->stream));
    return CRT_OK;
}

int crt_get_hit_info_device(crt_ctx* c, const crt_ray* d_rays, const crt_hit* d_hits, crt_hit_info* d_out, size_t n, void* stream)
{
    if (!c) return CRT_ERR_INVALID;
    const char* what = "crt_get_hit_info_device";
    int r;
    if ((r = shade_check(c, true, n, what))) return r;
    if (n == 0) return CRT_OK;
    HIPCK(c, hipSetDevice(c->cfg.device));
    if ((r = check_device_buffer(c, d_rays, n * sizeof(crt_ray), what)) || (r = check_device_buffer(c, d_hits, n * sizeof(crt_hit), what)) ||
        (r = check_device_buffer(c, d_out, n * sizeof(crt_hit_info), what))) return r;
    if (reinterpret_cast<uintptr_t>(d_out) & 15u) return c->fail(CRT_ERR_INVALID, "%s: the output buffer %p is not 16-byte aligned", what, (void*)d_out);
    hipStream_t st = nullptr; int k = 0;
    if ((r = begin_device_query(c, stream, what, &st, &k))) return r;
    HIPCK(c, crt_launch_hit_info(&c->hScene, d_rays, d_hits, d_out, (uint32_t)n, c->flat.objects, file_tri_count(c), st));
    return end_device_query(c, k, st);
}

int crt_get_sky_color(crt_ctx* c, const crt_ray* rays, float* rgb, size_t n)
{
    if (!c) return CRT_ERR_INVALID;
    int r;
    if ((r = shade_check(c, false, n, "crt_get_sky_color"))) return r;
    if (n == 0) return CRT_OK;
    if (!rays || !rgb) return c->fail(CRT_ERR_INVALID, "crt_get_sky_color: NULL buffer");
    if (c->havePrim) { memset(rgb, 0, n * 12); return CRT_OK; }
    HIPCK(c, hipSetDevice(c->cfg.device));
    if ((r = stage(c, n * (12 + sizeof(crt_ray))))) return r;
    float* dOut = reinterpret_cast<float*>(c->dStage); char* dRays = c->dStage + n * 12;
    HIPCK(c, hipMemcpyAsync(dRays, rays, n * sizeof(crt_ray), hipMemcpyHostToDevice, c->stream));
    HIPCK(c, crt_launch_sky_color(&c->hScene, dRays, dOut, (uint32_t)n, c->stream));
    HIPCK(c, hipMemcpyAsync(rgb, dOut, n * 12, hipMemcpyDeviceToHost, c->stream));
    HIPCK(c, hipStreamSynchronize(c->stream));
    return CRT_OK;
}

int crt_get_sky_color_device(crt_ctx* c, const crt_ray* d_rays, float* d_rgb, size_t n, void* stream)
{
    if (!c) return CRT_ERR_INVALID;
    const char* what = "crt_get_sky_color_device";
    int r;
    if ((r = shade_check(c, false, n, what))) return r;
    if (n == 0) return CRT_OK;
    HIPCK(c, hipSetDevice(c->cfg.device));
    if ((r = check_device_buffer(c, d_rays, n * sizeof(crt_ray), what)) || (r = check_device_buffer(c, d_rgb, n * 12, what))) return r;
    hipStream_t st = nullptr; int k = 0;
    if ((r = begin_device_query(c, stream, what, &st, &k))) return r;
    if (c->havePrim) HIPCK(c, hipMemsetAsync(d_rgb, 0, n * 12, st));
    else HIPCK(c, crt_launch_sky_color(&c->hScene, d_rays, d_rgb, (uint32_t)n, st));
    return end_device_query(c, k, st);
}

static int sample_check(crt_ctx* c, int accel, size_t n, const char* what)
{
    int r;
    if ((r = query_check(c, accel, false, n, what))) return r;
    const uint32_t words = sample_stack_words(c, accel);
    if (!sample_lds_fits(words)) return c->fail(CRT_ERR_UNSUPPORTED, "%s: a traversal stack of %u dwords per lane exceeds the kernel's LDS", what, words);
    return 0;
}

static hipError_t launch_sample(crt_ctx* c, int accel, const void* rays, uint32_t* seeds, float* rgb, uint32_t n, uint32_t* cursor, uint32_t* residentLanes, hipStream_t st)
{
    if (c->havePrim) return crt_launch_sample_query_prim(&c->hScene, &c->prim, rays, seeds, rgb, n, c->dCounters, cursor, residentLanes, st);
    return crt_launch_sample_query(accel, &c->hScene, &c->alt, accel ? &c->blasAlt[accel - 1] : nullptr, rays, seeds, rgb, n, c->dCounters, cursor, residentLanes, st);
}

int crt_sample(crt_ctx* c, int accel, const crt_ray* rays, uint32_t* seeds, float* rgb, size_t n)
{
    if (!c) return CRT_ERR_INVALID;
    int r;
    if ((r = sample_check(c, accel, n, "crt_sample"))) return r;
    if (n == 0) return CRT_OK;
    if (!rays || !seeds || !rgb) return c->fail(CRT_ERR_INVALID, "crt_sample: NULL buffer");
    HIPCK(c, hipSetDevice(c->cfg.device));
    if ((r = stage(c, n * (12 + sizeof(crt_ray) + 4)))) return r;
    float* dRgb = reinterpret_cast<float*>(c->dStage); char* dRays = c->dStage + n * 12; uint32_t* dSeeds = reinterpret_cast<uint32_t*>(dRays + n * sizeof(crt_ray));
    HIPCK(c, hipMemcpyAsync(dRays, rays, n * sizeof(crt_ray), hipMemcpyHostToDevice, c->stream));
    HIPCK(c, hipMemcpyAsync(dSeeds, seeds, n * 4, hipMemcpyHostToDevice, c->stream));
    HIPCK(c, launch_sample(c, accel, dRays, dSeeds, dRgb, (uint32_t)n, c->dQueryCursor, nullptr, c->stream));
    HIPCK(c, hipMemcpyAsync(rgb, dRgb, n * 12, hipMemcpyDeviceToHost, c->stream));
    HIPCK(c, hipMemcpyAsync(seeds, dSeeds, n * 4, hipMemcpyDeviceToHost, c->stream));
    HIPCK(c, hipStreamSynchronize(c->stream));
    return CRT_OK;
}

int crt_sample_device(crt_ctx* c, int accel, const crt_ray* d_rays, uint32_t* d_seeds, float* d_rgb, size_t n, void* stream)
{
    if (!c) return CRT_ERR_INVALID;
    const char* what = "crt_sample_device";
    int r;
    if ((r = sample_check(c, accel, n, what))) return r;
    if (n == 0) return CRT_OK;
    HIPCK(c, hipSetDevice(c->cfg.device));
    if ((r = check_device_buffer(c, d_rays, n * sizeof(crt_ray), what)) || (r = check_device_buffer(c, d_seeds, n * 4, what)) || (r = check_device_buffer(c, d_rgb, n * 12, what))) return r;
    hipStream_t st = nullptr; int k = 0;
    if ((r = begin_device_query(c, stream, what, &st, &k))) return r;
    if (accel != 0 && c->altReady) HIPCK(c, hipStreamWaitEvent(st, c->altReady, 0));
    HIPCK(c, launch_sample(c, accel, d_rays, d_seeds, d_rgb, (uint32_t)n, c->dQuerySlots + 16 * k, nullptr, st));
    return end_device_query(c, k, st);
}

extern "C" int crt_debug_sample_resident_lanes(crt_ctx* c, int accel, uint32_t* out)
{
    if (!c || !out) return CRT_ERR_INVALID;
    int r;
    if ((r = sample_check(c, accel, 0, "crt_debug_sample_resident_lanes"))) return r;
    HIPCK(c, hipSetDevice(c->cfg.device));
    HIPCK(c, launch_sample(c, accel, nullptr, nullptr, nullptr, 0u, nullptr, out, c->stream));
    return CRT_OK;
}

int crt_get_light(crt_ctx* c, float pos[3], float color[3])
{
    if (!c || !pos || !color) return CRT_ERR_INVALID;
    if (!c->haveScene) return c->fail(c->havePrim ? CRT_ERR_UNSUPPORTED : CRT_ERR_STATE, "crt_get_light needs a triangle scene (crt_upload_scene)");
    memcpy(pos, c->hScene.lightPos, 12);
    color[0] = 24.0f; color[1] = 24.0f; color[2] = 22.0f;
    return CRT_OK;
}

int crt_get_counters(crt_ctx* c, crt_counters* out)
{
    if (!c || !out) return CRT_ERR_INVALID;
    HIPCK(c, hipSetDevice(c->cfg.device));
    HIPCK(c, hipMemcpyAsync(out, c->dCounters, sizeof(crt::Counters), hipMemcpyDeviceToHost, c->stream));
    HIPCK(c, hipStreamSynchronize(c->stream));
    return CRT_OK;
}

int crt_reset_counters(crt_ctx* c)
{
    if (!c) return CRT_ERR_INVALID;
    HIPCK(c, hipSetDevice(c->cfg.device));
    HIPCK(c, hipMemsetAsync(c->dCounters, 0, sizeof(crt::Counters), c->stream));
    return CRT_OK;
}

int crt_get_timing(crt_ctx* c, crt_timing* out)
{
    if (!c || !out) return CRT_ERR_INVALID;
    HIPCK(c, hipSetDevice(c->cfg.device));
    HIPCK(c, hipStreamSynchronize(c->stream));
    for (auto st : c->streams) HIPCK(c, hipStreamSynchronize(st));
    if (c->aheadStream) HIPCK(c, hipStreamSynchronize(c->aheadStream));
    harvest_tuning(c);
    memset(out, 0, sizeof(*out));
    out->render_kernel_ms = (float)c->foldedRenderMs; out->resolve_kernel_ms = (float)c->foldedAccMs;
    for (auto& ev : c->evRender) { float ms = 0; HIPCK(c, hipEventElapsedTime(&ms, ev.a, ev.b)); out->render_kernel_ms += ms; }
    for (auto& ev : c->evAcc) { float ms = 0; HIPCK(c, hipEventElapsedTime(&ms, ev.a, ev.b)); out->resolve_kernel_ms += ms; }
    out->render_launches = (uint32_t)c->evRender.size() + c->foldedLaunches;
    out->pool_launches = c->poolLaunches; out->split_launches = c->splitLaunches;
    c->foldedRenderMs = c->foldedAccMs = 0; c->foldedLaunches = 0; c->poolLaunches = 0; c->splitLaunches = 0;
    for (auto& ev : c->evRender) c->evPool.push_back(ev);
    for (auto& ev : c->evAcc) c->evPool.push_back(ev);
    c->evRender.clear(); c->evAcc.clear();
    return CRT_OK;
}

int crt_get_tile_clocks(crt_ctx* c, uint64_t* out)
{
    if (!c || !out) return CRT_ERR_INVALID;
    if (!c->dTileClocks) return c->fail(CRT_ERR_STATE, "tile clocks are recorded only by a collectStats context");
    HIPCK(c, hipSetDevice(c->cfg.device));
    HIPCK(c, hipMemcpyAsync(out, c->dTileClocks, (size_t)c->tileCount * 16, hipMemcpyDeviceToHost, c->stream));
    HIPCK(c, hipStreamSynchronize(c->stream));
    return CRT_OK;
}

extern "C" int crt_debug_live_events(crt_ctx* c) { return c ? (int)(2 * (c->evRender.size() + c->evAcc.size() + c->evPool.size())) : -1; }

extern "C" int crt_debug_check_reciprocals(crt_ctx* c, uint64_t* out)
{
    if (!c || !out) return CRT_ERR_INVALID;
    HIPCK(c, hipSetDevice(c->cfg.device));
    unsigned long long* d = nullptr;
    HIPCK(c, hipMalloc(&d, 32));
    hipError_t e = hipMemsetAsync(d, 0, 32, c->stream);
    if (e == hipSuccess) e = crt_launch_check_reciprocals(d, c->stream);
    if (e == hipSuccess) e = hipMemcpyAsync(out, d, 32, hipMemcpyDeviceToHost, c->stream);
    if (e == hipSuccess) e = hipStreamSynchronize(c->stream);
    (void)hipFree(d);
    HIPCK(c, e);
    return CRT_OK;
}

extern "C" int crt_debug_device_probe(crt_ctx* c, int op, const void* in, void* out, uint32_t n)
{
    static const uint8_t words[17][2] = {{1, 1}, {1, 1}, {2, 1}, {1, 1}, {2, 1}, {6, 7}, {1, 18}, {4, 1}, {5, 3}, {13, 2}, {16, 4}, {2, 2}, {2, 2}, {2, 2}, {2, 2}, {4, 2}, {2, 1}};
    if (!c || !in || !out || op < 0 || op > 16 || n > (1u << 25)) return CRT_ERR_INVALID;
    if (n == 0) return CRT_OK;
    const size_t inBytes = (size_t)n * words[op][0] * 4, outBytes = (size_t)n * words[op][1] * 4;
    HIPCK(c, hipSetDevice(c->cfg.device));
    char* d = nullptr;
    HIPCK(c, hipMalloc((void**)&d, inBytes + outBytes));
    hipError_t e = hipMemcpyAsync(d, in, inBytes, hipMemcpyHostToDevice, c->stream);
    if (e == hipSuccess) e = (op <= 10) ? crt_launch_probe_f32(op, d, d + inBytes, n, c->stream) : crt_launch_probe_f64(op, d, d + inBytes, n, c->stream);
    if (e == hipSuccess) e = hipMemcpyAsync(out, d + inBytes, outBytes, hipMemcpyDeviceToHost, c->stream);
    if (e == hipSuccess) e = hipStreamSynchronize(c->stream);
    (void)hipFree(d);
    HIPCK(c, e);
    return CRT_OK;
}

extern "C" int crt_debug_plan_job(const uint32_t* cost, uint32_t n, uint32_t windows, uint32_t frames, int pool, double poolWindowTicks,
                                  uint32_t* table, uint32_t tableCap, uint32_t* head, uint32_t* order)
{
    if (!cost || !n || !table || !head || !order) return CRT_ERR_INVALID;
    crt_ctx c;
    c.tileCount = n; c.jobCostValid = true; c.poolWindowTicks = poolWindowTicks;
    c.streams.assign(2, nullptr);
    c.jobCost.assign(cost, cost + n);
    c.jobOrder.resize(n);
    for (uint32_t i = 0; i < n; i++) c.jobOrder[i] = i;
    std::stable_sort(c.jobOrder.begin(), c.jobOrder.end(), [&](uint32_t a, uint32_t b) { return c.jobCost[a] > c.jobCost[b]; });
    std::vector<uint32_t> t; uint32_t h = 0;
    plan_job(&c, windows, frames, pool != 0, t, &h);
    c.streams.clear();
    if (t.size() > tableCap) return CRT_ERR_INVALID;
    memcpy(table, t.data(), t.size() * 4); memcpy(order, c.jobOrder.data(), (size_t)n * 4); *head = h;
    return (int)t.size();
}

extern "C" int crt_debug_tile_costs(crt_ctx* c, uint32_t* out)
{
    if (!c || !out || !c->dTileCost) return CRT_ERR_INVALID;
    HIPCK(c, hipSetDevice(c->cfg.device));
    HIPCK(c, hipDeviceSynchronize());
    HIPCK(c, hipMemcpy(out, c->dTileCost, (size_t)c->tileCount * 4, hipMemcpyDeviceToHost));
    return CRT_OK;
}

extern "C" int crt_debug_lat_stage(crt_ctx* c, int stage, uint8_t* lanes, uint32_t* cost)
{
    if (!c || stage < 0 || stage > crt_ctx::kLatStages) return CRT_ERR_INVALID;
    if (c->latL[stage].size() != c->tileCount || c->latCost[stage].size() != c->tileCount) return CRT_ERR_STATE;
    if (lanes) memcpy(lanes, c->latL[stage].data(), c->tileCount);
    if (cost) memcpy(cost, c->latCost[stage].data(), (size_t)c->tileCount * 4);
    return c->latStage;
}

extern "C" int crt_debug_tile_stamps(crt_ctx* c, uint64_t* out)
{
    if (!c || !out || !c->dTileClocks) return CRT_ERR_INVALID;
    HIPCK(c, hipSetDevice(c->cfg.device));
    HIPCK(c, hipMemcpyAsync(out, c->dTileClocks + 2 * (size_t)c->tileCount, (size_t)c->tileCount * 128, hipMemcpyDeviceToHost, c->stream));
    HIPCK(c, hipStreamSynchronize(c->stream));
    return CRT_OK;
}

int crt_bind_accumulator(crt_ctx* c, void* p)
{
    if (!c) return CRT_ERR_INVALID;
    if (p && ((uintptr_t)p & 15u)) return c->fail(CRT_ERR_INVALID, "accumulator pointer must be 16-byte aligned");
    HIPCK(c, hipSetDevice(c->cfg.device));
    HIPCK(c, hipStreamSynchronize(c->stream));
    c->dAcc = p ? p : c->dAccOwned;
    return CRT_OK;
}

int crt_accumulator_device_ptr(crt_ctx* c, void** p)
{
    if (!c || !p) return CRT_ERR_INVALID;
    *p = c->dAcc; return CRT_OK;
}

}
```

### cpu-ray-tracer_amd/csrc/device/launch.h

```cpp
#pragma once
#include "layout.h"

#include <hip/hip_runtime.h>

extern "C" {

hipError_t crt_launch_check_reciprocals(unsigned long long* out, hipStream_t stream);
hipError_t crt_launch_render(const crt::Scene* sc, void* slab, crt::Counters* counters, unsigned long long* tileClocks, const uint32_t* tileOrder, uint32_t tileFirst, uint32_t tileStride,
    uint32_t tileCount, uint32_t tilesX, uint32_t sppFirst, uint32_t frames, uint32_t passes, uint32_t ldsBytes, int collectStats, const uint32_t* blockDesc, uint32_t nBlocks, uint32_t* tileCost,
    uint32_t rankCount, unsigned long long* launchClk, hipStream_t stream);
uint32_t crt_render_resident_waves(int device, int kind, uint32_t ldsBytes);
hipError_t crt_launch_accumulate(const void* slab, void* acc, uint32_t tileFirst, uint32_t tileStride, uint32_t tileCount, uint32_t tilesX, uint32_t W, uint32_t frames, uint32_t passes,
    hipStream_t stream);
hipError_t crt_launch_find_nearest(const crt::Scene* sc, const void* rays, void* hits, uint32_t n, crt::Counters* counters, uint32_t ldsBytes, uint32_t* cursor, hipStream_t stream);
hipError_t crt_launch_is_occluded(const crt::Scene* sc, const void* rays, int32_t* occluded, uint32_t n, uint32_t ldsBytes, uint32_t* cursor, hipStream_t stream);
hipError_t crt_launch_whitted(const crt::Scene* sc, int accel, const crt::AltAccelDev* alt, const crt::TlasAltDev* tl, void* acc, uint32_t* pixels, crt::Counters* counters, uint32_t ldsBytes,
    hipStream_t stream);
size_t crt_whitted_inspect_work_bytes(uint32_t pixelCount);
hipError_t crt_launch_whitted_inspect(const crt::Scene* sc, int accel, const crt::AltAccelDev* alt, const crt::TlasAltDev* tl, int inspect, int32_t peakIn, void* acc, uint32_t* pixels,
    crt::Counters* counters, int32_t* trav, int32_t* tested, void* work, uint32_t ldsBytes, hipStream_t stream);
hipError_t crt_launch_resolve(const void* acc, uint32_t* pixels, float* tileSums, uint32_t tileFirst, uint32_t tileStride, uint32_t tileCount, uint32_t tilesX, uint32_t W, float scale,
    hipStream_t stream);
hipError_t crt_launch_commit_frame(const void* slabWindow, uint32_t frameInWindow, uint32_t passes, void* acc, uint32_t* pixels, float* tileSums, uint32_t tileFirst, uint32_t tileStride,
    uint32_t tileCount, uint32_t tilesX, uint32_t W, float scale, hipStream_t stream);

uint32_t crt_pool_streams(uint32_t frames);
size_t crt_pool_scratch_bytes_per_window(uint32_t tileCount);
hipError_t crt_launch_render_pool(const crt::Scene* sc, void* slab, void* facScratch, crt::Counters* counters, unsigned long long* tileClocks, const uint32_t* tileOrder, uint32_t tileFirst,
    uint32_t tileStride, uint32_t tileCount, uint32_t tilesX, uint32_t sppFirst, uint32_t frames, uint32_t passes, int collectStats, uint32_t rankFirst, uint32_t* tileCost,
    unsigned long long* launchClk, hipStream_t stream);
int crt_debug_pool_stamps(unsigned long long* out, int reset);
int crt_debug_pool_density(unsigned long long* out, int reset);
size_t crt_debug_pool_timeline(unsigned long long* out, size_t cap);

uint32_t crt_probe_paths(void);
hipError_t crt_launch_probe(const crt::Scene* sc, uint32_t tileFirst, uint32_t tileStride, uint32_t tileCount, uint32_t tilesX, uint32_t* tileCost, hipStream_t stream);
hipError_t crt_launch_render_alt(int accel, const crt::Scene* sc, const crt::AltAccelDev* acc, const crt::TlasAltDev* tl, void* slab, crt::Counters* counters, uint32_t tileFirst, uint32_t tileStride,
    uint32_t tileCount, uint32_t tilesX, uint32_t sppFirst, uint32_t frames, uint32_t passes, hipStream_t stream);
hipError_t crt_launch_sample_query(int accel, const crt::Scene* sc, const crt::AltAccelDev* acc, const crt::TlasAltDev* tl, const void* rays, uint32_t* seeds, float* rgb, uint32_t n,
    crt::Counters* counters, uint32_t* cursor, uint32_t* residentLanes, hipStream_t stream);

hipError_t crt_launch_find_nearest_prim(const crt::PrimDev* p, const void* rays, void* hits, uint32_t n, hipStream_t stream);
hipError_t crt_launch_render_prim(const crt::Scene* sc, const crt::PrimDev* p, void* slab, crt::Counters* counters, uint32_t tileFirst, uint32_t tileStride, uint32_t tileCount, uint32_t tilesX,
    uint32_t sppFirst, uint32_t frames, uint32_t passes, hipStream_t stream);
hipError_t crt_launch_sample_query_prim(const crt::Scene* sc, const crt::PrimDev* p, const void* rays, uint32_t* seeds, float* rgb, uint32_t n, crt::Counters* counters, uint32_t* cursor,
    uint32_t* residentLanes, hipStream_t stream);
hipError_t crt_launch_probe_f64(int op, const void* in, void* out, uint32_t n, hipStream_t stream);

hipError_t crt_launch_find_nearest_alt(int kind, const crt::Scene* sc, const crt::AltAccelDev* acc, const void* rays, void* hits, uint32_t n, uint32_t* cursor, hipStream_t stream);
hipError_t crt_launch_is_occluded_alt(int kind, const crt::Scene* sc, const crt::AltAccelDev* acc, const void* rays, int32_t* occluded, uint32_t n, uint32_t* cursor, hipStream_t stream);
hipError_t crt_launch_tlas_alt_query(int kind, bool occl, const crt::Scene* sc, const crt::TlasAltDev* tl, const void* rays, void* out, uint32_t n, uint32_t* cursor, hipStream_t stream);

hipError_t crt_launch_hit_info(const crt::Scene* sc, const void* rays, const void* hits, void* out, uint32_t n, uint32_t objects, uint32_t fileTris, hipStream_t stream);
hipError_t crt_launch_sky_color(const crt::Scene* sc, const void* rays, float* rgb, uint32_t n, hipStream_t stream);
hipError_t crt_launch_refit(char* geom, uint32_t leafOff, uint32_t pairBase, uint32_t triBase, uint32_t triCount, const float* pos, const void* plan, const uint32_t* levelOff, uint32_t levels,
    uint32_t rootCode, float* out, hipStream_t stream);
hipError_t crt_launch_probe_f32(int op, const void* in, void* out, uint32_t n, hipStream_t stream);

hipError_t crt_launch_tlas_build(const char* geom, uint32_t instOff, const float* T, const float* rootBox, uint32_t blasCount, uint32_t pairRel, uint32_t instRel, void* out,
    hipStream_t stream);

uint32_t crt_debug_query_grid(void);

}

namespace crt {

inline uint32_t bounded_query_grid(uint32_t grid) { const uint32_t k = crt_debug_query_grid(); return (k != 0u && k < grid) ? k : grid; }

inline uint32_t query_grid(uint32_t n, uint32_t ldsBytes)
{
    uint32_t perCu = ldsBytes ? (160u * 1024u) / ldsBytes : 16u; if (perCu > 16u) perCu = 16u; if (perCu < 4u) perCu = 4u;
    const uint32_t need = (n + 63u) / 64u, fill = 256u * perCu;
    return bounded_query_grid(need < fill ? need : fill);
}

inline bool query_launch_begin(uint32_t n, uint32_t* cursor, hipStream_t stream, hipError_t* status)
{
    *status = hipSuccess;
    if (n == 0) return false;
    if (!cursor) { *status = hipErrorInvalidValue; return false; }
    if (hipMemsetAsync(cursor, 0, 4, stream) != hipSuccess) { *status = hipGetLastError(); return false; }
    return true;
}

}
```

### cpu-ray-tracer_amd/csrc/device/render_pool.hip

```cpp
#include "dev_common.h"
#include "launch.h"

namespace crt {

enum : uint32_t {
    F_OX = 0, F_OY, F_OZ, F_DX, F_DY, F_DZ,
    F_RX, F_RY, F_RZ,
    F_T,
    F_SEED, F_META,
    F_U, F_V,
    F_COUNT,
    F_CUR = F_U, F_PEND = F_V,
    F_TRI = F_RX
};
constexpr uint32_t kMetaItemMask = 0x7ffu, kMetaDepthShift = 11u, kMetaInside = 1u << 14, kMetaFresh = 1u << 15, kMetaObjShift = 16u, kMetaLowMask = 0xffffu;
constexpr uint32_t kQueueMask = 127u;

#ifndef CRT_POOL_MIN_WAVES
#define CRT_POOL_MIN_WAVES 4
#endif
#ifndef CRT_POOL_SHADE_MIN
#define CRT_POOL_SHADE_MIN 64
#endif
#ifndef CRT_POOL_NODE_STEPS
#define CRT_POOL_NODE_STEPS 2
#endif
#ifndef CRT_POOL_NODE2_MIN
#define CRT_POOL_NODE2_MIN 16
#endif
#ifndef CRT_POOL_STARVE
#define CRT_POOL_STARVE 40
#endif

#ifdef CRT_POOL_STAMPS
__device__ unsigned long long g_poolStamps[16];
#define CRT_PSTAMP(var) unsigned long long var; asm volatile("s_memtime %0\n\ts_waitcnt lgkmcnt(0)" : "=s"(var) :: "memory")
#define CRT_PACC(i, a, b) (pst[i] += (b) - (a))
#else
#define CRT_PSTAMP(var)
#define CRT_PACC(i, a, b)
#endif
#ifdef CRT_POOL_DENS
__device__ unsigned long long g_poolDens[32];
#define CRT_DENS(i, v) (dens[i] += (uint32_t)(v))
#define CRT_DENS_MASK(i, pred) (dens[i] += (uint32_t)__popcll(__builtin_amdgcn_ballot_w64(pred)))
#else
#define CRT_DENS(i, v)
#define CRT_DENS_MASK(i, pred)
#endif
#ifdef CRT_POOL_TIMELINE
__device__ unsigned long long* g_poolTimeline = nullptr;
#endif
__device__ __forceinline__ bool lane_in(uint64_t m) { return __builtin_amdgcn_inverse_ballot_w64(m); }
__device__ __forceinline__ uint64_t finite3_mask(f3 v)
{
    const uint32_t m = 0x7f800000u;
    return __builtin_amdgcn_ballot_w64((asu(v.x) & m) != m) & __builtin_amdgcn_ballot_w64((asu(v.y) & m) != m) & __builtin_amdgcn_ballot_w64((asu(v.z) & m) != m);
}
__device__ __forceinline__ uint32_t rank_in(uint64_t m) { return __builtin_amdgcn_mbcnt_hi((uint32_t)(m >> 32), __builtin_amdgcn_mbcnt_lo((uint32_t)m, 0u)); }

template <int KIND, bool COUNT, int S>
__global__ __launch_bounds__(64, CRT_POOL_MIN_WAVES) void render_pool_kernel(const Scene sc, float4* __restrict__ slab, float* __restrict__ facScratch, Counters* __restrict__ counters,
                                                             unsigned long long* __restrict__ tileClocks, const uint32_t* __restrict__ tileOrder,
                                                             uint32_t tileFirst, uint32_t tileStride, uint32_t tileCount, uint32_t tilesX,
                                                             uint32_t sppFirst, uint32_t frames, uint32_t passes, uint32_t groups, uint32_t rankFirst, uint32_t* __restrict__ tileCost, unsigned long long* __restrict__ launchClk)
{
    extern __shared__ uint32_t lds[];
    const uint32_t lane = threadIdx.x;
#ifdef CRT_POOL_TIMELINE
    const unsigned long long tl0 = wall_clock64();
#endif
    const unsigned long long clk0 = (COUNT || tileCost) ? wall_clock64() : 0ull;
    if (launchClk && lane == 0) { atomicMax(&launchClk[0], ~clk0); atomicMax(&launchClk[1], clk0); }
    const uint32_t rank0 = blockIdx.x / groups, grp = blockIdx.x - rank0 * groups, rank = rank0 + rankFirst;
    if (rank >= tileCount) return;
    const uint32_t tl = tileOrder ? tileOrder[rank] : rank;
    const uint32_t frame0 = grp * (uint32_t)S;
    const uint32_t nStreams = (frames - frame0 < (uint32_t)S) ? frames - frame0 : (uint32_t)S;
    const uint32_t tile = tileFirst + tl * tileStride;
    const uint32_t tx = tile % tilesX, ty = tile / tilesX;
    const char* __restrict__ geom = sc.geom;
    float* __restrict__ fac = facScratch + (size_t)blockIdx.x * (15u * (uint32_t)S);

    char* const ldsB = reinterpret_cast<char*>(lds);
    const uint32_t laneB = lane * 2u;
    uint32_t* st = lds + (sc.stackDepth + 1u) * 32u;
    float* stf = reinterpret_cast<float*>(st);
    uint8_t* qEnd = reinterpret_cast<uint8_t*>(st + F_COUNT * S);
    uint8_t* qBnc = qEnd + 128, * qRdy = qEnd + 256;
    auto stk_top = [&](uint32_t at) -> uint32_t { return *reinterpret_cast<const uint16_t*>(ldsB + at); };
    auto stk_put = [&](uint32_t at, uint32_t v) { *reinterpret_cast<uint16_t*>(ldsB + at) = (uint16_t)v; };

    Cnt cn; cn.rays = cn.primary = cn.interior = cn.leaf = cn.tri = cn.tlas = cn.visits = cn.meshhits = 0;
    uint32_t trips = 0;
#ifdef CRT_POOL_DENS
    uint32_t dens[32]; for (int i = 0; i < 32; i++) dens[i] = 0;
#endif
    const uint32_t items = 256u * passes;
    const uint32_t rowLen = 64u * passes;
    const f3 nil3 = mk3(0.0f, 0.0f, 0.0f);

    for (uint32_t s = lane; s < nStreams; s += 64u) {
        st[F_SEED * S + s] = init_seed(tx + ty * (uint32_t)sc.W + (sppFirst + (frame0 + s) * passes) * 1799u);
        st[F_META * S + s] = kMetaFresh;
        qEnd[s] = (uint8_t)s;
    }
    uint32_t endH = 0, endT = nStreams, bncH = 0, bncT = 0, rdyH = 0, rdyT = 0;

    uint64_t mRes = 0ull;
    uint64_t mFinite = ~0ull;
    uint32_t sid = 0, cur = kRefDone, spB = laneB, metaLo = 0u;
    f3 tO = nil3, tD = nil3, trD = nil3;
    Hit h; h.t = 1e34f; h.u = 0; h.v = 0; h.objIdx = -1; h.triIdx = -1;
    rec4 q0 = {0, 0, 0, 0}, q1 = q0, q2 = q0, q3 = q0;

    auto new_ray = [&](bool act, uint32_t s, f3 v, bool norm, f3 O, uint32_t seed, uint32_t meta) {
        f3 D = v, rD = v; Hit nh; nh.t = 1e34f; nh.u = 0; nh.v = 0; nh.objIdx = -1; nh.triIdx = -1;
        uint32_t ncur = kRefDone, pend = 0u;
        if (act) {
            const float inv = rcp_exact(__builtin_sqrtf(dot3(v, v)));
            D = norm ? v * inv : v;
            rD = rcp_exact3(D);
            cn.rays++;
            {
                const kernarg_f lp = scene_floats(offsetof(Scene, lightInvT));
                const kernarg_f ax = scene_floats(offsetof(Scene, lightAxis));
                LightFloor lf;
#pragma unroll
                for (int i = 0; i < 12; i++) lf.lightInvT[i] = lp[i];
                lf.lightSize = lp[15]; lf.floorN[0] = lp[19]; lf.floorN[1] = lp[20]; lf.floorN[2] = lp[21]; lf.floorD = lp[22];
                lf.lightAxis = asu(ax[0]); lf.floorAxisY = asu(ax[1]);
                hit_light_floor(lf, O, D, nh);
            }
            if (sc.rootIsPair) {
                const kernarg_f rp = scene_floats(offsetof(Scene, rootPair));
                const rec4 a0 = {rp[0], rp[1], rp[2], rp[3]}, a1 = {rp[4], rp[5], rp[6], rp[7]};
                const rec4 b0 = {rp[8], rp[9], rp[10], rp[11]}, b1 = {rp[12], rp[13], rp[14], rp[15]};
                float d1, d2;
                if (__builtin_amdgcn_ballot_w64(!finite3(rD)) == 0ull) { d1 = box_fast(a0, a1, O, rD, nh.t); d2 = box_fast(b0, b1, O, rD, nh.t); }
                else { d1 = box_exact(a0, a1, O, rD, nh.t); d2 = box_exact(b0, b1, O, rD, nh.t); }
                const bool sw = d1 > d2;
                const float dn = sw ? d2 : d1, df = sw ? d1 : d2;
                const uint32_t rn = sw ? asu(b1.w) : asu(a1.w), rf = sw ? asu(a1.w) : asu(b1.w);
                const bool hitN = dn != 1e30f;
                pend = (hitN && df != 1e30f) ? rf : 0u;
                ncur = hitN ? rn : kRefDone;
                if (COUNT) { if (KIND == 0) cn.interior++; else cn.tlas++; }
            } else ncur = sc.rootRef16;
            if (COUNT && KIND == 0 && (ncur & kRef16TagMask) == 0u && ncur != kRefDone) cn.leaf++;
            stf[F_OX * S + s] = O.x; stf[F_OY * S + s] = O.y; stf[F_OZ * S + s] = O.z;
            stf[F_DX * S + s] = D.x; stf[F_DY * S + s] = D.y; stf[F_DZ * S + s] = D.z;
            stf[F_RX * S + s] = rD.x; stf[F_RY * S + s] = rD.y; stf[F_RZ * S + s] = rD.z;
            stf[F_T * S + s] = nh.t;
            st[F_SEED * S + s] = seed; st[F_META * S + s] = meta | ((uint32_t)(nh.objIdx + 1) << kMetaObjShift);
            st[F_CUR * S + s] = ncur; st[F_PEND * S + s] = pend;
        }
        const uint32_t depth = (meta >> kMetaDepthShift) & 7u;
        const uint64_t mAct = __builtin_amdgcn_ballot_w64(act);
        const uint64_t mW = mAct & __builtin_amdgcn_ballot_w64(ncur != kRefDone);
        const uint64_t mStop = __builtin_amdgcn_ballot_w64((uint32_t)(nh.objIdx + 1) <= 1u) | __builtin_amdgcn_ballot_w64((int)depth >= sc.depthLimit);
        const uint64_t mE = mAct & ~mW & mStop, mB = mAct & ~mW & ~mStop;
        CRT_DENS(20, __popcll(mAct)); CRT_DENS(19, __popcll(mW));
        if (lane_in(mW)) qRdy[(rdyT + rank_in(mW)) & kQueueMask] = (uint8_t)s;
        if (lane_in(mE)) qEnd[(endT + rank_in(mE)) & kQueueMask] = (uint8_t)s;
        if (lane_in(mB)) qBnc[(bncT + rank_in(mB)) & kQueueMask] = (uint8_t)s;
        rdyT += (uint32_t)__popcll(mW); endT += (uint32_t)__popcll(mE); bncT += (uint32_t)__popcll(mB);
    };
    auto world_ray = [&]() {
        tO = mk3(stf[F_OX * S + sid], stf[F_OY * S + sid], stf[F_OZ * S + sid]);
        tD = mk3(stf[F_DX * S + sid], stf[F_DY * S + sid], stf[F_DZ * S + sid]);
        trD = mk3(stf[F_RX * S + sid], stf[F_RY * S + sid], stf[F_RZ * S + sid]);
    };

    uint64_t mNode2 = 0ull;
    auto node_step = [&](uint64_t m) {
        const bool allFinite = (m & ~mFinite) == 0ull;
        if (lane_in(m)) {
            if (COUNT) { if (KIND == 1 && (cur & kRef16TlasBit) != 0u) cn.tlas++; else cn.interior++; }
            const uint32_t top = stk_top(spB);
            float d1, d2;
            if (__builtin_expect(allFinite, 1)) { d1 = box_fast(q0, q1, tO, trD, h.t); d2 = box_fast(q2, q3, tO, trD, h.t); }
            else { d1 = box_exact(q0, q1, tO, trD, h.t); d2 = box_exact(q2, q3, tO, trD, h.t); }
            const bool sw = d1 > d2;
            const float dn = sw ? d2 : d1, df = sw ? d1 : d2;
            const uint32_t rn = sw ? asu(q3.w) : asu(q1.w), rf = sw ? asu(q1.w) : asu(q3.w);
            stk_put(spB + 128u, rf);
            const bool hitN = dn != 1e30f, push = hitN && df != 1e30f;
            const bool pop = !hitN && spB != laneB;
            cur = hitN ? rn : (pop ? top : kRefDone);
            spB = spB + (push ? 128u : 0u) - (pop ? 128u : 0u);
            if (COUNT && (cur & kRef16TagMask) == 0u && cur != kRefDone) cn.leaf++;
        }
    };
    auto load_records = [&](uint64_t m) {
        const uint32_t idx = cur & kRef16IndexMask;
        const bool inter = (cur & kRef16Interior) != 0u;
        uint32_t oa = idx * (inter ? 64u : 48u) + (inter ? 0u : sc.leafOff - 48u);
        if (KIND == 1 && (cur & kRef16TlasBit) != 0u)
            oa = (cur & kRef16Interior) ? sc.instOff + idx * 128u : sc.tlasPairOff + idx * 64u;
        if (lane_in(m)) { q0 = ldg(geom, oa); q1 = ldg(geom, oa + 16u); q2 = ldg(geom, oa + 32u); q3 = ldg(geom, oa + 48u); }
    };

    auto tri_step = [&](uint64_t m) {
        CRT_DENS(3, 1); CRT_DENS(4, __popcll(m));
        if (lane_in(m)) {
            if (COUNT) cn.tri++;
            const uint32_t top = stk_top(spB);
            hit_tri(q0, q1, q2, tO, tD, h);
            const bool more = asu(q2.w) > 1u;
            const bool pop = !more && spB != laneB;
            const uint32_t next = more ? cur + 1u : (pop ? top : kRefDone);
            spB -= pop ? 128u : 0u;
            if (COUNT && !more && (next & kRef16TagMask) == 0u && next != kRefDone) cn.leaf++;
            cur = next;
        }
    };

#ifdef CRT_POOL_STAMPS
    unsigned long long pst[12] = {0, 0, 0, 0, 0, 0, 0, 0, 0, 0, 0, 0};
#endif
    for (;;) {
        CRT_PSTAMP(p0);
        if (mRes != 0ull) {
            uint64_t mNode, mTlas = 0ull;
            if (KIND == 0) mNode = mRes & __builtin_amdgcn_ballot_w64(cur > 0x7fffu);
            else { mTlas = mRes & __builtin_amdgcn_ballot_w64(cur >= kRef16TlasLeaf); mNode = mRes & __builtin_amdgcn_ballot_w64(cur - kRef16TlasBit < 0x8000u); }
            const uint64_t mTri = mRes & ~(mNode | mTlas);
            asm volatile("" : "+v"(q0), "+v"(q1), "+v"(q2), "+v"(q3));
            CRT_DENS(22, __popcll(mRes));
            if (mNode) { CRT_DENS(1, 1); CRT_DENS(2, __popcll(mNode)); }

            if (KIND == 1 && mTlas) { CRT_DENS(23, 1); CRT_DENS(24, __popcll(mTlas)); }
            uint64_t mBack = 0ull;
            if (KIND == 1 && mTlas != 0ull) {
                if (lane_in(mTlas)) {
                    if (COUNT) { cn.tlas++; cn.visits++; }
                    const f3 O = mk3(stf[F_OX * S + sid], stf[F_OY * S + sid], stf[F_OZ * S + sid]);
                    const f3 D = mk3(stf[F_DX * S + sid], stf[F_DY * S + sid], stf[F_DZ * S + sid]);
                    to_object_space(q0, q1, q2, O, D, tO, tD, trD);
                    spB += 128u; stk_put(spB, kRef16Return);
                    const uint32_t next = asu(q3.y);
                    if (COUNT && (next & kRef16TagMask) == 0u && next != kRefDone) cn.leaf++;
                    cur = next;
                }
                mFinite = (mFinite & ~mTlas) | (mTlas & finite3_mask(trD));
            }
            if (mNode != 0ull) node_step(mNode);
#if CRT_POOL_NODE_STEPS > 1
            uint64_t mLeafNow = 0ull;
#pragma unroll
            for (int rep = 1; rep < CRT_POOL_NODE_STEPS; rep++) {
                const uint64_t mStepped = rep == 1 ? mNode : mNode2;
                mNode2 = mStepped & (KIND == 0 ? __builtin_amdgcn_ballot_w64(cur > 0x7fffu) : __builtin_amdgcn_ballot_w64(cur - kRef16TlasBit < 0x8000u));
                if ((uint32_t)__popcll(mNode2) < (uint32_t)CRT_POOL_NODE2_MIN) { mNode2 = 0ull; break; }
                const uint64_t mLeaf = mStepped & __builtin_amdgcn_ballot_w64((cur & kRef16TagMask) == 0u) & ~__builtin_amdgcn_ballot_w64(cur == kRefDone);
                load_records(mNode2 | mLeaf);
                mLeafNow |= mLeaf;
                CRT_DENS(28, 1); CRT_DENS(29, __popcll(mNode2));
                node_step(mNode2);
            }
            const uint64_t mTriAll = mTri | mLeafNow;
            const uint64_t mTriRan = mTriAll;
#else
            const uint64_t mTriAll = mTri;
            const uint64_t mTriRan = mTriAll;
#endif
            if (mTriAll != 0ull) tri_step(mTriAll);
            if (KIND == 1) {
                mBack = (mNode | mTriRan) & __builtin_amdgcn_ballot_w64(cur == kRef16Return);
                if (mBack != 0ull) {
                    if (lane_in(mBack)) {
                        world_ray();
                        const bool pop = spB != laneB;
                        const uint32_t top = stk_top(spB);
                        cur = pop ? top : kRefDone; spB -= pop ? 128u : 0u;
                        if (COUNT && (cur & kRef16TagMask) == 0u && cur != kRefDone) cn.leaf++;
                    }
                    mFinite = (mFinite & ~mBack) | (mBack & finite3_mask(trD));
                }
            }
            asm volatile("" ::: "memory");
            const uint64_t mFin = mRes & __builtin_amdgcn_ballot_w64(cur == kRefDone);
            if (mFin != 0ull) {
                CRT_DENS(5, 1); CRT_DENS(6, __popcll(mFin));
                const uint32_t depth = (metaLo >> kMetaDepthShift) & 7u;
                const uint64_t mStop = __builtin_amdgcn_ballot_w64((uint32_t)(h.objIdx + 1) <= 1u) | __builtin_amdgcn_ballot_w64((int)depth >= sc.depthLimit);
                const uint64_t mE = mFin & mStop, mB = mFin & ~mStop;
                if (lane_in(mFin)) {
                    stf[F_T * S + sid] = h.t; stf[F_U * S + sid] = h.u; stf[F_V * S + sid] = h.v;
                    st[F_TRI * S + sid] = (uint32_t)h.triIdx;
                    st[F_META * S + sid] = metaLo | ((uint32_t)(h.objIdx + 1) << kMetaObjShift);
                }
                if (lane_in(mE)) qEnd[(endT + rank_in(mE)) & kQueueMask] = (uint8_t)sid;
                if (lane_in(mB)) qBnc[(bncT + rank_in(mB)) & kQueueMask] = (uint8_t)sid;
                endT += (uint32_t)__popcll(mE); bncT += (uint32_t)__popcll(mB);
                mRes &= ~mFin;
            }
            asm volatile("" ::: "memory");
        }
        CRT_PSTAMP(p1); CRT_PACC(0, p0, p1);
        if (__builtin_expect(mRes == 0ull, 0)) {
            if ((endT - endH) + (bncT - bncH) + (rdyT - rdyH) == 0u) break;
        }
        if (COUNT) trips++;
        CRT_DENS(0, 1);
        {
            const uint32_t nRdy = rdyT - rdyH;
            const uint64_t mFree = ~mRes;
            if (nRdy != 0u) if (mFree != 0ull) {
                const uint32_t myRank = rank_in(mFree);
                const uint64_t mTake = mFree & __builtin_amdgcn_ballot_w64(myRank < nRdy);
                CRT_DENS(7, 1); CRT_DENS(8, __popcll(mTake));
                if (lane_in(mTake)) {
                    sid = qRdy[(rdyH + myRank) & kQueueMask];
                    tO = mk3(stf[F_OX * S + sid], stf[F_OY * S + sid], stf[F_OZ * S + sid]);
                    tD = mk3(stf[F_DX * S + sid], stf[F_DY * S + sid], stf[F_DZ * S + sid]);
                    trD = mk3(stf[F_RX * S + sid], stf[F_RY * S + sid], stf[F_RZ * S + sid]);
                    const uint32_t meta = st[F_META * S + sid];
                    h.t = stf[F_T * S + sid]; h.objIdx = (int)(meta >> kMetaObjShift) - 1; h.u = 0; h.v = 0; h.triIdx = -1;
                    metaLo = meta & kMetaLowMask;
                    cur = st[F_CUR * S + sid];
                    const uint32_t pend = st[F_PEND * S + sid];
                    stk_put(laneB + 128u, pend);
                    spB = laneB + (pend ? 128u : 0u);
                }
                mFinite = (mFinite & ~mTake) | (mTake & finite3_mask(trD));
                mRes |= mTake;
                rdyH += (uint32_t)__popcll(mTake);
            }
            if (mRes != 0ull) {
                CRT_DENS(21, 1);
                const uint32_t idx = cur & kRef16IndexMask;
                const bool inter = (cur & kRef16Interior) != 0u;
                uint32_t oa = idx * (inter ? 64u : 48u) + (inter ? 0u : sc.leafOff - 48u);
                if (KIND == 1 && (cur & kRef16TlasBit) != 0u)
                    oa = (cur & kRef16Interior) ? sc.instOff + idx * 128u : sc.tlasPairOff + idx * 64u;
                if (!lane_in(mRes)) oa = 0u;
                q0 = ldg(geom, oa); q1 = ldg(geom, oa + 16u); q2 = ldg(geom, oa + 32u); q3 = ldg(geom, oa + 48u);
            }
        }
        asm volatile("" ::: "memory");
        {
            const uint32_t nEnd = endT - endH, nBnc = bncT - bncH, nRdy = rdyT - rdyH, nRes = (uint32_t)__popcll(mRes);
            const bool starving = nRes + nRdy < (uint32_t)CRT_POOL_STARVE;
            bool runEnd = false, runBnc = false;
            if ((nEnd | nBnc) >= (uint32_t)CRT_POOL_SHADE_MIN || starving) {
                runEnd = nEnd >= (uint32_t)CRT_POOL_SHADE_MIN || (starving && nEnd > 0u && nEnd >= nBnc);
                runBnc = nBnc >= (uint32_t)CRT_POOL_SHADE_MIN || (starving && nBnc > nEnd);
            }

            CRT_PSTAMP(p2b); CRT_PACC(1, p1, p2b);
            if (runEnd) {
                const uint32_t n = nEnd < 64u ? nEnd : 64u;
                const bool act = lane < n;
                const uint32_t s = act ? qEnd[(endH + lane) & kQueueMask] : 0u;
                endH += n;
                uint32_t meta = 0, seed = 0; int obj = -1; f3 D = nil3;
                if (act) { meta = st[F_META * S + s]; seed = st[F_SEED * S + s]; obj = (int)(meta >> kMetaObjShift) - 1; D = mk3(stf[F_DX * S + s], stf[F_DY * S + s], stf[F_DZ * S + s]); }
                const bool first = (meta & kMetaFresh) != 0u;
                const int depth = (int)((meta >> kMetaDepthShift) & 7u);
                uint32_t item = meta & kMetaItemMask;
                const bool ended = act && !first, miss = ended && obj == -1;
                CRT_DENS(9, 1); CRT_DENS(10, n); CRT_DENS_MASK(11, miss); CRT_DENS_MASK(13, act && first); CRT_DENS_MASK(25, ended && depth > 0); CRT_DENS_MASK(26, ended && depth > 1); CRT_DENS_MASK(27, ended && depth > 2);
                if (ended && obj >= 2) cn.meshhits++;
                float fk[15];
#pragma unroll
                for (int k = 0; k < 5; k++) {
                    fk[3 * k] = fk[3 * k + 1] = fk[3 * k + 2] = 0.0f;
                    if (ended && depth > k) {
#pragma unroll
                        for (int j = 0; j < 3; j++) fk[3 * k + j] = __hip_atomic_load(fac + (3 * k + j) * S + s, __ATOMIC_RELAXED, __HIP_MEMORY_SCOPE_AGENT);
                    }
                }
                uint32_t skyTexel = 0u;
                if (miss) {
                    const float phi = crt_atan2f(-D.z, D.x) + CRT_PI, theta = crt_acosf(-D.y);
                    const kernarg_f sk = scene_floats(offsetof(Scene, skyOffset));
                    skyTexel = sc.texels[tex_index(asu(sk[0]), (int)asu(sk[1]), (int)asu(sk[2]), phi * CRT_INV2PI, theta * CRT_INVPI)];
                }
                bool gen = act && first;
                size_t sampleAt = 0;
                if (ended) {
                    uint32_t pix = item, pass = 0;
                    if (passes != 1u) { pix = item / passes; pass = item - pix * passes; }
                    const uint32_t fr = frame0 + s;
                    sampleAt = (((size_t)(fr >> 6) * tileCount + tl) * 256u + pix) * rowLen + ((fr & 63u) * passes + pass);
                    item++;
                    gen = item < items;
                }
                const kernarg_f cam = scene_floats(offsetof(Scene, camPos));
                const f3 camPos = mk3(cam[0], cam[1], cam[2]);
                f3 v = camPos;
                if (gen) {
                    const uint32_t pix = (passes == 1u) ? item : item / passes;
                    const int x = (int)(tx * 16u + (pix & 15u)), y = (int)(ty * 16u + (pix >> 4));
                    const float jy = rnd(seed);
                    const float jx = rnd(seed);
                    const float u = ((float)x + jx) * cam[12], vv = ((float)y + jy) * cam[13];
                    const f3 TL = mk3(cam[3], cam[4], cam[5]), TR = mk3(cam[6], cam[7], cam[8]), BL = mk3(cam[9], cam[10], cam[11]);
                    const f3 P = TL + u * (TR - TL) + vv * (BL - TL);
                    v = P - camPos;
                    cn.primary++;
                }
                CRT_DENS_MASK(12, gen);
                CRT_PSTAMP(e1); CRT_PACC(2, p2b, e1);
                new_ray(gen, s, v, true, camPos, seed, item);
                CRT_PSTAMP(e2); CRT_PACC(3, e1, e2);
                if (ended) {
                    f3 L = miss ? tex_unpack(skyTexel) : ((depth >= sc.depthLimit) ? mk3(0, 0, 0) : mk3(24, 24, 22));
#pragma unroll
                    for (int k = 4; k >= 0; k--)
                        if (depth > k) L = mk3(fk[3 * k], fk[3 * k + 1], fk[3 * k + 2]) * L;
                    slab[sampleAt] = make_float4(L.x, L.y, L.z, 0.0f);
                }
#ifdef CRT_POOL_STAMPS
                { CRT_PSTAMP(e3); CRT_PACC(4, e2, e3); pst[10]++; }
#endif
                asm volatile("" :: "v"(fk[0]), "v"(fk[1]), "v"(fk[2]), "v"(fk[3]), "v"(fk[4]), "v"(fk[5]), "v"(fk[6]), "v"(fk[7]), "v"(fk[8]), "v"(fk[9]), "v"(fk[10]), "v"(fk[11]), "v"(fk[12]), "v"(fk[13]), "v"(fk[14]), "v"(skyTexel));
            }
            CRT_PSTAMP(p3);
            asm volatile("" ::: "memory");
            if (runBnc) {
                const uint32_t n = nBnc < 64u ? nBnc : 64u;
                const bool act = lane < n;
                const uint32_t s = act ? qBnc[(bncH + lane) & kQueueMask] : 0u;
                bncH += n;
                f3 O = nil3, D = nil3; float ht = 0, hu = 0, hv = 0; int obj = 1; uint32_t tri = 0, seed = 0, meta = 0;
                if (act) {
                    tri = st[F_TRI * S + s];
                    O = mk3(stf[F_OX * S + s], stf[F_OY * S + s], stf[F_OZ * S + s]);
                    D = mk3(stf[F_DX * S + s], stf[F_DY * S + s], stf[F_DZ * S + s]);
                    ht = stf[F_T * S + s]; hu = stf[F_U * S + s]; hv = stf[F_V * S + s];
                    seed = st[F_SEED * S + s]; meta = st[F_META * S + s]; obj = (int)(meta >> kMetaObjShift) - 1;
                }
                const bool mesh = act && obj >= 2;
                CRT_DENS(14, 1); CRT_DENS(15, n); CRT_DENS_MASK(16, mesh);
                rec4 s0 = {0, 0, 0, 0}, s1 = s0, s2 = s0, s3 = s0;
                if (mesh) { const uint32_t so = sc.shadeOff + tri * 64u; s0 = ldg(geom, so); s1 = ldg(geom, so + 16u); s2 = ldg(geom, so + 32u); s3 = ldg(geom, so + 48u); cn.meshhits++; }
                const bool inside = (meta & kMetaInside) != 0u;
                const int depth = (int)((meta >> kMetaDepthShift) & 7u);
                const uint32_t item = meta & kMetaItemMask;
                float tu = 0, tv = 0; uint32_t tOff = 0; int tW = 0, tH = 0;
                f3 I = O, N = O, absorb = O; float refl = 0, refr = 0;
                f3 v = O, pre = O; bool norm = false, diffuse = false, newInside = false;
                if (act) {
                    I = O + ht * D;
                    if (obj == 1) {
                        const kernarg_f fl = scene_floats(offsetof(Scene, floorN));
                        const kernarg_f fm = scene_floats(offsetof(Scene, floorMat));
                        N = mk3(fl[0], fl[1], fl[2]);
                        if (N.y == 1) {
                            float u = I.x, vv = I.z;
                            u *= fl[4]; vv *= fl[4];
                            tu = u - __builtin_floorf(u); tv = vv - __builtin_floorf(vv);
                        }
                        refl = fm[0]; refr = fm[1];
                        absorb = mk3(fm[2], fm[3], fm[4]);
                        tOff = asu(fm[5]); tW = (int)asu(fm[6]); tH = (int)asu(fm[7]);
                    } else {
                        const f3 n0 = mk3(s0.x, s0.y, s0.z), n1 = mk3(s0.w, s1.x, s1.y), n2 = mk3(s1.z, s1.w, s2.x);
                        const float w = 1 - hu - hv;
                        const f3 Nn = w * n0 + hu * n1 + hv * n2;
                        tu = w * s2.y + hu * s2.w + hv * s3.y;
                        tv = w * s2.z + hu * s3.x + hv * s3.z;
                        const rec4* mp = reinterpret_cast<const rec4*>(sc.mats + (int)asu(s3.w));
                        const rec4 m0 = mp[0], m1 = mp[1];
                        refl = m0.x; refr = m0.y; absorb = mk3(m0.z, m0.w, m1.x);
                        tOff = asu(m1.y); tW = (int)asu(m1.z); tH = (int)asu(m1.w);
                        if (KIND == 0) {
                            N = normalize3(Nn);
                        } else {
                            const uint32_t io = sc.instOff + (uint32_t)(obj - 2) * 128u + 64u;
                            const rec4 r0 = ldg(geom, io), r1 = ldg(geom, io + 16), r2 = ldg(geom, io + 32);
                            N = normalize3(mk3(r0.x * Nn.x + r0.y * Nn.y + r0.z * Nn.z + r0.w * 0.0f,
                                               r1.x * Nn.x + r1.y * Nn.y + r1.z * Nn.z + r1.w * 0.0f,
                                               r2.x * Nn.x + r2.y * Nn.y + r2.z * Nn.z + r2.w * 0.0f));
                        }
                    }
                    if (dot3(N, D) > 0) N = -N;
                    uint32_t texel = 0x00ffffffu;
                    if (tW > 0) texel = sc.texels[tex_index(tOff, tW, tH, tu, tv)];
                    f3 medium = mk3(1, 1, 1);
                    if (inside) {
                        const f3 ab = absorb * -ht;
                        medium = mk3(crt_expf(ab.x), crt_expf(ab.y), crt_expf(ab.z));
                    }
                    CRT_PSTAMP(b1); CRT_PACC(5, p3, b1);
                    const float r = rnd(seed);
                    const bool mirror = r < refl, dielectric = !mirror && r < refl + refr;
                    if (mirror) {
                        v = D - 2.0f * N * dot3(N, D);
                    } else if (dielectric) {
                        v = D - 2.0f * N * dot3(N, D);
                        const float n1 = inside ? 1.2f : 1, n2 = inside ? 1 : 1.2f;
                        const float eta = n1 / n2, cosi = dot3(-D, N);
                        const float cost2 = 1.0f - eta * eta * (1 - cosi * cosi);
                        if (cost2 > 0) {
                            const float a = n1 - n2, b2 = n1 + n2, R0 = (a * a) / (b2 * b2), cc = 1 - cosi;
                            const float Fr = R0 + (1 - R0) * (cc * cc * cc * cc * cc);
                            const f3 T = eta * D + ((eta * cosi - __builtin_sqrtf(__builtin_fabsf(cost2))) * N);
                            if (rnd(seed) > Fr) { v = T; newInside = !inside; }
                        }
                    } else {
                        f3 Rr;
                        do {
                            const float rz = rnd_pm1(seed);
                            const float ry = rnd_pm1(seed);
                            const float rx = rnd_pm1(seed);
                            Rr = mk3(rx, ry, rz);
                        } while (dot3(Rr, Rr) > 1);
                        if (dot3(Rr, N) < 0) Rr = Rr * -1.0f;
                        v = Rr; norm = true; diffuse = true;
                    }
                    const f3 c = (tW > 0) ? tex_unpack(texel) : mk3(1.0f, 1.0f, 1.0f);
                    if (diffuse) {
                        const f3 brdf = c * CRT_INVPI;
                        pre = medium * brdf * 2.0f * CRT_PI;
                    } else pre = c * medium;
                    CRT_PSTAMP(b2); CRT_PACC(6, b1, b2);
                    const float inv = rcp_exact(__builtin_sqrtf(dot3(v, v)));
                    const f3 nv = norm ? v * inv : v;
                    v = nv;
                    const f3 factor = diffuse ? pre * dot3(nv, N) : pre;
                    float* fd = fac + (3 * depth) * S + s;
                    __hip_atomic_store(fd, factor.x, __ATOMIC_RELAXED, __HIP_MEMORY_SCOPE_AGENT);
                    __hip_atomic_store(fd + S, factor.y, __ATOMIC_RELAXED, __HIP_MEMORY_SCOPE_AGENT);
                    __hip_atomic_store(fd + 2 * S, factor.z, __ATOMIC_RELAXED, __HIP_MEMORY_SCOPE_AGENT);
                    O = I + nv * CRT_EPS;
                    CRT_PSTAMP(b3); CRT_PACC(7, b2, b3);
                }
                CRT_PSTAMP(b4);
                new_ray(act, s, v, false, O, seed, item | ((uint32_t)(depth + 1) << kMetaDepthShift) | (newInside ? kMetaInside : 0u));
#ifdef CRT_POOL_STAMPS
                { CRT_PSTAMP(b5); CRT_PACC(8, b4, b5); pst[11]++; }
#endif
                asm volatile("" :: "v"(s0), "v"(s1), "v"(s2), "v"(s3));
            }
#ifdef CRT_POOL_STAMPS
            pst[9]++;
#endif
        }
    }
#ifdef CRT_POOL_STAMPS
    if (lane == 0) for (int i = 0; i < 12; i++) atomicAdd(&g_poolStamps[i], pst[i]);
#endif
#ifdef CRT_POOL_DENS
    if (lane == 0) for (int i = 0; i < 32; i++) if (dens[i]) atomicAdd(&g_poolDens[i], (unsigned long long)dens[i]);
#endif

#ifdef CRT_POOL_TIMELINE
    if (lane == 0 && g_poolTimeline) { uint32_t hw; asm volatile("s_getreg_b32 %0, hwreg(HW_REG_HW_ID)" : "=s"(hw)); g_poolTimeline[3 * (size_t)blockIdx.x] = tl0; g_poolTimeline[3 * (size_t)blockIdx.x + 1] = wall_clock64(); g_poolTimeline[3 * (size_t)blockIdx.x + 2] = hw; }
#endif
    if (tileCost && lane == 0 && nStreams == (uint32_t)S) atomicMax(&tileCost[tl], (uint32_t)((wall_clock64() - clk0) * 64ull / (uint32_t)S));
    if (launchClk && lane == 0) { const unsigned long long now = wall_clock64(), last = __hip_atomic_load(&launchClk[1], __ATOMIC_RELAXED, __HIP_MEMORY_SCOPE_AGENT), from = last > clk0 ? last : clk0; if (now > from) atomicAdd(&launchClk[2], now - from); }
    if (COUNT && tileClocks && lane == 0 && groups == 1u) {
        tileClocks[2 * tl] = wall_clock64() - clk0;
        tileClocks[2 * tl + 1] = trips;
    }
    uint32_t vals[8] = {cn.rays, cn.primary, cn.interior, cn.leaf, cn.tri, cn.tlas, cn.visits, cn.meshhits};
#pragma unroll
    for (int i = 0; i < 8; i++) {
        if (!COUNT && i >= 2 && i != 7) continue;
        uint32_t sum = wave_sum(vals[i]);
        if (lane == 0 && sum) atomicAdd(&counters->v[i], (unsigned long long)sum);
    }
}

}

#ifndef CRT_POOL_STREAMS
#define CRT_POOL_STREAMS 128
#endif
extern "C" uint32_t crt_pool_streams(uint32_t frames) { return frames > 64u ? (uint32_t)CRT_POOL_STREAMS : 64u; }
#ifndef CRT_POOL_EXTRA_LDS
#define CRT_POOL_EXTRA_LDS 0
#endif
extern "C" uint32_t crt_pool_lds_bytes(uint32_t stackDepth, uint32_t streams) { return (stackDepth + 1u) * 64u * 2u + crt::F_COUNT * streams * 4u + 3u * 128u + (uint32_t)CRT_POOL_EXTRA_LDS; }
extern "C" size_t crt_pool_scratch_bytes_per_window(uint32_t tileCount) { return (size_t)tileCount * 128u * 15u * 4u; }

#ifdef CRT_POOL_STAMPS
extern "C" int crt_debug_pool_stamps(unsigned long long* out, int reset)
{
    if (out && hipMemcpyFromSymbol(out, HIP_SYMBOL(crt::g_poolStamps), 128) != hipSuccess) return -1;
    if (reset) { unsigned long long z[16] = {}; if (hipMemcpyToSymbol(HIP_SYMBOL(crt::g_poolStamps), z, 128) != hipSuccess) return -1; }
    return 0;
}
#endif
#ifdef CRT_POOL_DENS
extern "C" int crt_debug_pool_density(unsigned long long* out, int reset)
{
    if (out && hipMemcpyFromSymbol(out, HIP_SYMBOL(crt::g_poolDens), 256) != hipSuccess) return -1;
    if (reset) { unsigned long long z[32] = {}; if (hipMemcpyToSymbol(HIP_SYMBOL(crt::g_poolDens), z, 256) != hipSuccess) return -1; }
    return 0;
}
#endif
#ifdef CRT_POOL_TIMELINE
static unsigned long long* g_timelineHost = nullptr; static size_t g_timelineCount = 0;
extern "C" size_t crt_debug_pool_timeline(unsigned long long* out, size_t cap)
{
    const size_t n = g_timelineCount < cap ? g_timelineCount : cap;
    if (out && n) (void)hipMemcpy(out, g_timelineHost, n * 24, hipMemcpyDeviceToHost);
    return g_timelineCount;
}
#endif
extern "C" hipError_t crt_launch_render_pool(const crt::Scene* sc, void* slab, void* facScratch, crt::Counters* counters, unsigned long long* tileClocks, const uint32_t* tileOrder,
                                             uint32_t tileFirst, uint32_t tileStride, uint32_t tileCount, uint32_t tilesX, uint32_t sppFirst,
                                             uint32_t frames, uint32_t passes, int collectStats, uint32_t rankFirst, uint32_t* tileCost, unsigned long long* launchClk, hipStream_t stream)
{
    if (tileCount == 0 || frames == 0) return hipSuccess;
    if (!sc->ref16ok) return hipErrorInvalidValue;
    const uint32_t S = crt_pool_streams(frames);
    const uint32_t groups = (frames + S - 1u) / S;
    if ((unsigned long long)tileCount * groups > 0x7fffffffull) return hipErrorInvalidValue;
    if (rankFirst >= tileCount) return hipSuccess;
    dim3 grid((tileCount - rankFirst) * groups), block(64);
#ifdef CRT_POOL_TIMELINE
    { static unsigned long long* buf = nullptr; static size_t cap = 0;
      if (cap < (size_t)grid.x) { if (buf) (void)hipFree(buf); (void)hipMalloc((void**)&buf, (size_t)grid.x * 24); cap = grid.x; (void)hipMemcpyToSymbol(HIP_SYMBOL(crt::g_poolTimeline), &buf, sizeof(buf)); }
      (void)hipMemsetAsync(buf, 0, (size_t)grid.x * 24, stream); g_timelineHost = buf; g_timelineCount = grid.x; }
#endif
    const uint32_t ldsBytes = crt_pool_lds_bytes(sc->stackDepth, S);
#define CRT_LAUNCH(K, C, SS) hipLaunchKernelGGL((crt::render_pool_kernel<K, C, SS>), grid, block, ldsBytes, stream, *sc, (float4*)slab, (float*)facScratch, counters, tileClocks, tileOrder, tileFirst, tileStride, tileCount, tilesX, sppFirst, frames, passes, groups, rankFirst, tileCost, launchClk)
#define CRT_LAUNCH_S(K, C) do { if (S == 64u) CRT_LAUNCH(K, C, 64); else CRT_LAUNCH(K, C, CRT_POOL_STREAMS); } while (0)
    if (sc->kind == 0) { if (collectStats) CRT_LAUNCH_S(0, true); else CRT_LAUNCH_S(0, false); }
    else { if (collectStats) CRT_LAUNCH_S(1, true); else CRT_LAUNCH_S(1, false); }
#undef CRT_LAUNCH_S
#undef CRT_LAUNCH
    return hipGetLastError();
}
```

Before: 29650 Mrays/s.

## Let pool wavefronts own multiple frame groups per tile, refilling streams from a cost plan

Adds a host-side planner that uses measured per-tile costs to give cheap, late-starting tiles wavefronts owning 2-8x more frames for the first part of the job. Inside the kernel, a stream that finishes a frame is refilled with the next unowned frame through an LDS slot-to-frame map, and blocks are located with a binary search over a wave table. The aim is fewer, longer wavefronts and lower per-wave startup cost while keeping the makespan balanced. The cost is extra LDS, more kernel arguments and branches, and reliance on cost estimates that may be wrong. The plan is only used after the job-cost trial, which picks whichever variant measured faster.

Result: faster. 30140 Mrays/s, median of 6 (+1.6%).

```diff
diff --git a/cpu-ray-tracer_amd/csrc/abi.cpp b/cpu-ray-tracer_amd/csrc/abi.cpp
--- a/cpu-ray-tracer_amd/csrc/abi.cpp
+++ b/cpu-ray-tracer_amd/csrc/abi.cpp
@@ -118,6 +118,7 @@
     uint32_t* dJobDesc = nullptr; uint32_t* hJobDesc = nullptr; uint32_t jobDescCap = 0, jobBlocks = 0, jobHead = 0; hipEvent_t jobDescReady = nullptr;
     uint32_t planWindows = 0, planFrames = 0; bool planPool = false, planValid = false;
     double jobTrialMs[2] = {0, 0};
+    uint32_t jobWaveOff = 0, jobWaveBlocks = 0, jobLongFrames = 0, jobLongWaves = 0, lastLongWaves = 0;
     std::vector<hipEvent_t> splitEvents;
     size_t splitSeq = 0; uint32_t splitLaunches = 0;
     uint64_t poolMinWaves = 65000;
@@ -1199,6 +1200,65 @@
     *head = pool ? h : 0u;
 }
 
+struct PoolWaveTerms { double poolLong = 2.4, load = 1.0, safety = 1.0, guard = 12.0, share = 1.0; };
+static uint64_t pool_wave_plan(const uint32_t* cost, uint32_t nr, uint32_t frames, uint32_t S, double perCost, double startTicks, uint32_t resident, const PoolWaveTerms& tm,
+                               std::vector<uint32_t>& wf, uint32_t* longFrames, std::vector<double>* start, double* aimOut)
+{
+    wf.assign(nr, S); *longFrames = 0;
+    if (start) start->assign(nr, 0.0);
+    if (aimOut) *aimOut = 0;
+    const uint64_t perTile = (frames + S - 1u) / S, plain = (uint64_t)nr * perTile;
+    if (!cost || S <= 64u || nr == 0u) return plain;
+    const uint32_t F1 = (uint32_t)((double)frames * std::min(tm.share, 1.0)) / (8u * S) * (8u * S);
+    if (F1 == 0u) return plain;
+    double aim = startTicks, m = startTicks;
+    std::vector<double> st(nr);
+    for (uint32_t r = 0; r < nr; r++) { st[r] = m; m += (double)(F1 / 64u) * (double)cost[r] * perCost; aim += (double)((frames + 63u) / 64u) * (double)cost[r] * perCost; }
+    if (start) *start = st;
+    if (aimOut) *aimOut = aim;
+    if ((double)plain < tm.guard * (double)resident) return plain;
+    const uint64_t shortWaves = (uint64_t)nr * ((frames - F1 + S - 1u) / S);
+    for (int kMax = 3; kMax >= 1; kMax--) {
+        uint64_t waves = shortWaves; bool any = false;
+        for (uint32_t r = 0; r < nr; r++) {
+            int k = kMax;
+            while (k > 0 && st[r] + tm.safety * tm.poolLong * tm.load * (double)cost[r] * (double)((uint64_t)S << k) / 128.0 > aim) k--;
+            wf[r] = S << k; any = any || k > 0;
+            waves += F1 / wf[r];
+        }
+        if (!any) break;
+        if ((double)waves >= tm.guard * (double)resident) { *longFrames = F1; return waves; }
+    }
+    wf.assign(nr, S);
+    return plain;
+}
+static uint32_t pool_wave_table(const std::vector<uint32_t>& wf, uint32_t longFrames, uint32_t S, std::vector<uint32_t>& tab, uint32_t* longWaves)
+{
+    tab.resize(2 * wf.size()); uint32_t b = 0, lw = 0;
+    for (size_t r = 0; r < wf.size(); r++) {
+        tab[2 * r] = b; tab[2 * r + 1] = wf[r];
+        b += longFrames / wf[r];
+        if (wf[r] > S) lw += longFrames / wf[r];
+    }
+    if (longWaves) *longWaves = lw;
+    return b;
+}
+static bool pool_wave_terms(PoolWaveTerms& tm)
+{
+    if (const char* e = hook("CRT_POOL_REFILL_SAFETY")) { const double v = atof(e); if (v > 0) tm.safety = v; }
+    if (const char* e = hook("CRT_POOL_REFILL_GUARD")) { const double v = atof(e); if (v > 0) tm.guard = v; }
+    if (const char* e = hook("CRT_POOL_REFILL_SHARE")) { const double v = atof(e); if (v > 0) tm.share = v; }
+    return !hook("CRT_POOL_REFILL_OFF");
+}
+static uint32_t forced_wave_frames(uint32_t S)
+{
+    const char* e = hook("CRT_POOL_WAVE_FRAMES");
+    if (!e) return 0u;
+    const long v = atol(e);
+    if (v < (long)S) return S;
+    return (uint32_t)std::min<long>(v, 8192) / S * S;
+}
+
 static int install_job_plan(crt_ctx* c, uint32_t windows, uint32_t frames, bool pool)
 {
     if (c->planValid && c->planWindows == windows && c->planFrames == frames && c->planPool == pool) return 0;
@@ -1206,6 +1266,33 @@
     plan_job(c, windows, frames, pool, table, &head);
     c->planValid = true; c->planWindows = windows; c->planFrames = frames; c->planPool = pool; c->jobHead = head; c->jobBlocks = (uint32_t)table.size();
     c->jobTrialMs[0] = c->jobTrialMs[1] = 0;
+    c->jobWaveOff = c->jobWaveBlocks = c->jobLongFrames = c->jobLongWaves = 0;
+    PoolWaveTerms terms;
+    const uint32_t S = crt_pool_streams(frames);
+    if (pool && c->jobCostValid && !c->cfg.collectStats && head < c->tileCount && pool_wave_terms(terms) && !forced_wave_frames(S)) {
+        const uint32_t nr = c->tileCount - head;
+        std::vector<uint32_t> cost(nr), wf, tab;
+        double costSum = 0; for (uint32_t v : c->jobCost) costSum += (double)v;
+        const double perCost = (c->poolWindowTicks > 0 && costSum > 0) ? c->poolWindowTicks / costSum : 1.0 / 4096.0;
+        double startTicks = 0;
+        for (uint32_t r = 0; r < head; r++) startTicks += (double)windows * 1.2 * (double)c->jobCost[c->jobOrder[r]] * perCost;
+        for (uint32_t r = 0; r < nr; r++) cost[r] = c->jobCost[c->jobOrder[head + r]];
+        double aim = 0; uint32_t F1 = 0, lw = 0, blocks = 0;
+        pool_wave_plan(cost.data(), nr, frames, S, perCost, startTicks, 4096u, terms, wf, &F1, nullptr, &aim);
+        if (F1) blocks = pool_wave_table(wf, F1, S, tab, &lw);
+        if (lw) {
+            c->jobWaveOff = (uint32_t)table.size(); c->jobWaveBlocks = blocks; c->jobLongFrames = F1; c->jobLongWaves = lw;
+            table.insert(table.end(), tab.begin(), tab.end());
+        }
+        if (hook("CRT_LAT_VERBOSE")) {
+            uint32_t cnt[4] = {0, 0, 0, 0}; double share[4] = {0, 0, 0, 0}, sum = 0;
+            for (uint32_t r = 0; r < nr; r++) { int k = 0; while ((S << k) < wf[r]) k++; cnt[k]++; share[k] += cost[r]; sum += cost[r]; }
+            fprintf(stderr, "[crt] pool launch of %u ranks x %u frames: aim %.1f ms, most expensive tile %.2f ms, long part %u frames in %u wavefronts, %u of them own more than %u frames (safety %.2f, guard %.1f x 4096, share %.2f); tiles by frames per wavefront (share of the cost):",
+                    nr, frames, aim * 1e-5, nr ? cost[0] * 1e-5 : 0.0, F1, blocks, lw, S, terms.safety, terms.guard, terms.share);
+            for (int k = 0; k < 4; k++) fprintf(stderr, " %u: %u (%.3f)", S << k, cnt[k], sum > 0 ? share[k] / sum : 0.0);
+            fprintf(stderr, "\n");
+        }
+    }
     if (table.empty()) return 0;
     if (c->jobDescCap < table.size()) {
         if (c->dJobDesc) (void)hipFree(c->dJobDesc);
@@ -1229,6 +1316,7 @@
     const uint32_t* blockDesc = nullptr; uint32_t nBlocks = 0;
     bool wantCost = false, wantJobCost = false, pool = false;
     uint32_t head = 0, jobBlocks = 0; unsigned long long* jobClk = nullptr;
+    uint32_t waveFrames = 0, waveBlocks = 0, longFrames = 0, longWaves = 0; const uint32_t* waveTab = nullptr;
 };
 
 static int next_block_table(crt_ctx* c);
@@ -1279,18 +1367,23 @@
     if (L.nf > 64u && c->jobCostValid) {
         if ((r = install_job_plan(c, L.windows, L.nf, L.pool))) return r;
         int use = 1;
-        if (c->jobBlocks && !hook("CRT_PLAN_NO_TRIAL")) {
+        if ((c->jobBlocks || c->jobLongWaves) && !hook("CRT_PLAN_NO_TRIAL")) {
             if (c->jobTrialMs[1] > 0 && c->jobTrialMs[0] > 0) use = c->jobTrialMs[1] <= c->jobTrialMs[0] ? 1 : 0;
             else if (c->jobTrialMs[1] > 0 && c->jobTrialMs[0] == 0) use = 0;
             c->evRender.back().mode = 100 + use;
         }
-        if (use) { L.head = c->jobHead; L.jobBlocks = c->jobBlocks; }
-    }
-    if (L.jobBlocks) HIPCK(c, hipStreamWaitEvent(L.st, c->jobDescReady, 0));
+        if (use) { L.head = c->jobHead; L.jobBlocks = c->jobBlocks; if (L.pool && c->jobLongWaves) { L.waveTab = c->dJobDesc + c->jobWaveOff; L.waveBlocks = c->jobWaveBlocks; L.longFrames = c->jobLongFrames; L.longWaves = c->jobLongWaves; } }
+    }
+    if (L.pool) if (const uint32_t S = crt_pool_streams(L.nf); const uint32_t n = forced_wave_frames(S)) {
+        L.waveFrames = n; L.waveTab = nullptr; L.waveBlocks = 0;
+        L.longWaves = n > S ? (c->tileCount - L.head) * (L.nf / n + ((L.nf % n) > S ? 1u : 0u)) : 0u;
+    }
+    if (L.jobBlocks || L.waveTab) HIPCK(c, hipStreamWaitEvent(L.st, c->jobDescReady, 0));
     if (L.wantJobCost) {
         L.jobClk = reinterpret_cast<unsigned long long*>(reinterpret_cast<char*>(c->dJobCost) + job_cost_clk_offset(c));
         c->recPool = L.pool; c->recWindows = L.windows;
-        c->recWaves = L.pool ? c->tileCount * ((L.nf + crt_pool_streams(L.nf) - 1u) / crt_pool_streams(L.nf)) : c->tileCount * L.windows;
+        const uint32_t perWave = L.pool ? std::max(crt_pool_streams(L.nf), L.waveFrames) : 64u;
+        c->recWaves = L.pool ? c->tileCount * ((L.nf + perWave - 1u) / perWave) : c->tileCount * L.windows;
         c->recResident = L.pool ? 4096u : 5120u;
     }
     return 0;
@@ -1321,7 +1414,9 @@
         }
         if (le == hipSuccess)
             le = crt_launch_render_pool(&c->hScene, L.slab, scratch, c->dCounters, c->dTileClocks, c->dTileOrder, c->tileFirst, c->tileStride, c->tileCount, (uint32_t)c->tilesX,
-                                        L.sppFirst, L.nf, L.passes, c->cfg.collectStats, L.jobBlocks ? L.head : 0u, L.wantJobCost ? c->dJobCost : nullptr, L.jobClk, st2);
+                                        L.sppFirst, L.nf, L.passes, c->cfg.collectStats, L.jobBlocks ? L.head : 0u, L.waveFrames, L.waveTab, L.waveBlocks, L.longFrames,
+                                        L.wantJobCost ? c->dJobCost : nullptr, L.jobClk, st2);
+        if (le == hipSuccess) c->lastLongWaves = L.longWaves;
         if (L.jobBlocks && le == hipSuccess) le = join(st2);
     } else if (L.jobBlocks) {
         le = launch_table(c->dJobDesc, L.jobBlocks, nullptr);
@@ -2412,6 +2507,20 @@
     return (int)t.size();
 }
 
+extern "C" long long crt_debug_pool_wave_plan(const uint32_t* cost, uint32_t nr, uint32_t frames, double perCost, double startTicks, uint32_t resident, double safety, double guard,
+                                              double share, uint32_t* wf, uint32_t* longFrames, double* start, double* aim)
+{
+    if (!nr || !frames || !wf || !longFrames) return CRT_ERR_INVALID;
+    PoolWaveTerms tm; if (safety > 0) tm.safety = safety; if (guard > 0) tm.guard = guard; if (share > 0) tm.share = share;
+    std::vector<uint32_t> w; std::vector<double> st;
+    const uint64_t waves = pool_wave_plan(cost, nr, frames, crt_pool_streams(frames), perCost, startTicks, resident, tm, w, longFrames, &st, aim);
+    memcpy(wf, w.data(), (size_t)nr * 4);
+    if (start) memcpy(start, st.data(), (size_t)nr * 8);
+    return (long long)waves;
+}
+extern "C" int crt_debug_pool_long_waves(crt_ctx* c) { return c ? (int)c->lastLongWaves : -1; }
+extern "C" void crt_debug_pool_wave_terms(double* out) { const PoolWaveTerms tm; out[0] = tm.poolLong; out[1] = tm.load; out[2] = tm.safety; out[3] = tm.guard; out[4] = tm.share; }
+
 extern "C" int crt_debug_tile_costs(crt_ctx* c, uint32_t* out)
 {
     if (!c || !out || !c->dTileCost) return CRT_ERR_INVALID;
diff --git a/cpu-ray-tracer_amd/csrc/device/launch.h b/cpu-ray-tracer_amd/csrc/device/launch.h
--- a/cpu-ray-tracer_amd/csrc/device/launch.h
+++ b/cpu-ray-tracer_amd/csrc/device/launch.h
@@ -27,8 +27,9 @@
 uint32_t crt_pool_streams(uint32_t frames);
 size_t crt_pool_scratch_bytes_per_window(uint32_t tileCount);
 hipError_t crt_launch_render_pool(const crt::Scene* sc, void* slab, void* facScratch, crt::Counters* counters, unsigned long long* tileClocks, const uint32_t* tileOrder, uint32_t tileFirst,
-    uint32_t tileStride, uint32_t tileCount, uint32_t tilesX, uint32_t sppFirst, uint32_t frames, uint32_t passes, int collectStats, uint32_t rankFirst, uint32_t* tileCost,
-    unsigned long long* launchClk, hipStream_t stream);
+    uint32_t tileStride, uint32_t tileCount, uint32_t tilesX, uint32_t sppFirst, uint32_t frames, uint32_t passes, int collectStats, uint32_t rankFirst, uint32_t waveFrames,
+    const uint32_t* waveTab, uint32_t tabBlocks, uint32_t longFrames, uint32_t* tileCost, unsigned long long* launchClk, hipStream_t stream);
+uint32_t crt_pool_lds_bytes(uint32_t stackDepth, uint32_t streams);
 int crt_debug_pool_stamps(unsigned long long* out, int reset);
 int crt_debug_pool_density(unsigned long long* out, int reset);
 size_t crt_debug_pool_timeline(unsigned long long* out, size_t cap);
diff --git a/cpu-ray-tracer_amd/csrc/device/render_pool.hip b/cpu-ray-tracer_amd/csrc/device/render_pool.hip
--- a/cpu-ray-tracer_amd/csrc/device/render_pool.hip
+++ b/cpu-ray-tracer_amd/csrc/device/render_pool.hip
@@ -41,9 +41,10 @@
 #define CRT_PACC(i, a, b)
 #endif
 #ifdef CRT_POOL_DENS
-__device__ unsigned long long g_poolDens[32];
+__device__ unsigned long long g_poolDens[48];
 #define CRT_DENS(i, v) (dens[i] += (uint32_t)(v))
 #define CRT_DENS_MASK(i, pred) (dens[i] += (uint32_t)__popcll(__builtin_amdgcn_ballot_w64(pred)))
+#define CRT_LIVE_BUCKET(n) ((n) >= 112u ? 0u : (n) >= 96u ? 1u : (n) >= 64u ? 2u : 3u)
 #else
 #define CRT_DENS(i, v)
 #define CRT_DENS_MASK(i, pred)
@@ -63,7 +64,8 @@
 __global__ __launch_bounds__(64, CRT_POOL_MIN_WAVES) void render_pool_kernel(const Scene sc, float4* __restrict__ slab, float* __restrict__ facScratch, Counters* __restrict__ counters,
                                                              unsigned long long* __restrict__ tileClocks, const uint32_t* __restrict__ tileOrder,
                                                              uint32_t tileFirst, uint32_t tileStride, uint32_t tileCount, uint32_t tilesX,
-                                                             uint32_t sppFirst, uint32_t frames, uint32_t passes, uint32_t groups, uint32_t rankFirst, uint32_t* __restrict__ tileCost, unsigned long long* __restrict__ launchClk)
+                                                             uint32_t sppFirst, uint32_t frames, uint32_t passes, uint32_t groups, uint32_t waveFrames, const uint32_t* __restrict__ waveTab, uint32_t tabBlocks, uint32_t longFrames,
+                                                             uint32_t rankFirst, uint32_t* __restrict__ tileCost, unsigned long long* __restrict__ launchClk)
 {
     extern __shared__ uint32_t lds[];
     const uint32_t lane = threadIdx.x;
@@ -72,11 +74,21 @@
 #endif
     const unsigned long long clk0 = (COUNT || tileCost) ? wall_clock64() : 0ull;
     if (launchClk && lane == 0) { atomicMax(&launchClk[0], ~clk0); atomicMax(&launchClk[1], clk0); }
-    const uint32_t rank0 = blockIdx.x / groups, grp = blockIdx.x - rank0 * groups, rank = rank0 + rankFirst;
+    uint32_t rank0, grp, wf = waveFrames, first = 0u, limit = frames;
+    if (waveTab) {
+        if (blockIdx.x < tabBlocks) {
+            uint32_t lo = 0u, hi = tileCount - rankFirst;
+            while (hi - lo > 1u) { const uint32_t mid = (lo + hi) >> 1; if (waveTab[2u * mid] <= blockIdx.x) lo = mid; else hi = mid; }
+            rank0 = lo; grp = blockIdx.x - waveTab[2u * lo]; wf = waveTab[2u * lo + 1u]; limit = longFrames;
+        } else { const uint32_t b = blockIdx.x - tabBlocks; rank0 = b / groups; grp = b - rank0 * groups; wf = (uint32_t)S; first = longFrames; }
+    } else { rank0 = blockIdx.x / groups; grp = blockIdx.x - rank0 * groups; }
+    const uint32_t rank = rank0 + rankFirst;
     if (rank >= tileCount) return;
     const uint32_t tl = tileOrder ? tileOrder[rank] : rank;
-    const uint32_t frame0 = grp * (uint32_t)S;
-    const uint32_t nStreams = (frames - frame0 < (uint32_t)S) ? frames - frame0 : (uint32_t)S;
+    const uint32_t frame0 = first + grp * wf;
+    if (frame0 >= limit) return;
+    const uint32_t nOwn = (limit - frame0 < wf) ? limit - frame0 : wf;
+    const uint32_t nStreams = nOwn < (uint32_t)S ? nOwn : (uint32_t)S;
     const uint32_t tile = tileFirst + tl * tileStride;
     const uint32_t tx = tile % tilesX, ty = tile / tilesX;
     const char* __restrict__ geom = sc.geom;
@@ -88,13 +100,15 @@
     float* stf = reinterpret_cast<float*>(st);
     uint8_t* qEnd = reinterpret_cast<uint8_t*>(st + F_COUNT * S);
     uint8_t* qBnc = qEnd + 128, * qRdy = qEnd + 256;
+    uint16_t* slotFrame = reinterpret_cast<uint16_t*>(qEnd + 384);
     auto stk_top = [&](uint32_t at) -> uint32_t { return *reinterpret_cast<const uint16_t*>(ldsB + at); };
     auto stk_put = [&](uint32_t at, uint32_t v) { *reinterpret_cast<uint16_t*>(ldsB + at) = (uint16_t)v; };
 
     Cnt cn; cn.rays = cn.primary = cn.interior = cn.leaf = cn.tri = cn.tlas = cn.visits = cn.meshhits = 0;
     uint32_t trips = 0;
 #ifdef CRT_POOL_DENS
-    uint32_t dens[32]; for (int i = 0; i < 32; i++) dens[i] = 0;
+    uint32_t dens[48]; for (int i = 0; i < 48; i++) dens[i] = 0;
+    uint32_t live = nStreams; unsigned long long liveClk = wall_clock64();
 #endif
     const uint32_t items = 256u * passes;
     const uint32_t rowLen = 64u * passes;
@@ -104,7 +118,9 @@
         st[F_SEED * S + s] = init_seed(tx + ty * (uint32_t)sc.W + (sppFirst + (frame0 + s) * passes) * 1799u);
         st[F_META * S + s] = kMetaFresh;
         qEnd[s] = (uint8_t)s;
+        if (S > 64) slotFrame[s] = (uint16_t)s;
     }
+    uint32_t nextFrame = nStreams;
     uint32_t endH = 0, endT = nStreams, bncH = 0, bncT = 0, rdyH = 0, rdyT = 0;
 
     uint64_t mRes = 0ull;
@@ -304,6 +320,9 @@
         }
         if (COUNT) trips++;
         CRT_DENS(0, 1);
+#ifdef CRT_POOL_DENS
+        dens[32u + CRT_LIVE_BUCKET(live)]++;
+#endif
         {
             const uint32_t nRdy = rdyT - rdyH;
             const uint64_t mFree = ~mRes;
@@ -361,6 +380,9 @@
                 const int depth = (int)((meta >> kMetaDepthShift) & 7u);
                 uint32_t item = meta & kMetaItemMask;
                 const bool ended = act && !first, miss = ended && obj == -1;
+#ifdef CRT_POOL_DENS
+                dens[36u + CRT_LIVE_BUCKET(live)]++;
+#endif
                 CRT_DENS(9, 1); CRT_DENS(10, n); CRT_DENS_MASK(11, miss); CRT_DENS_MASK(13, act && first); CRT_DENS_MASK(25, ended && depth > 0); CRT_DENS_MASK(26, ended && depth > 1); CRT_DENS_MASK(27, ended && depth > 2);
                 if (ended && obj >= 2) cn.meshhits++;
                 float fk[15];
@@ -383,11 +405,30 @@
                 if (ended) {
                     uint32_t pix = item, pass = 0;
                     if (passes != 1u) { pix = item / passes; pass = item - pix * passes; }
-                    const uint32_t fr = frame0 + s;
+                    const uint32_t fr = frame0 + (S > 64 ? (uint32_t)slotFrame[s] : s);
                     sampleAt = (((size_t)(fr >> 6) * tileCount + tl) * 256u + pix) * rowLen + ((fr & 63u) * passes + pass);
                     item++;
                     gen = item < items;
                 }
+                if (S > 64) if (nextFrame < nOwn) {
+                    const uint64_t mDone = __builtin_amdgcn_ballot_w64(ended) & ~__builtin_amdgcn_ballot_w64(gen);
+                    if (mDone != 0ull) {
+                        const uint32_t f = nextFrame + rank_in(mDone);
+                        const uint64_t mTake = mDone & __builtin_amdgcn_ballot_w64(f < nOwn);
+                        if (lane_in(mTake)) {
+                            slotFrame[s] = (uint16_t)f;
+                            seed = init_seed(tx + ty * (uint32_t)sc.W + (sppFirst + (frame0 + f) * passes) * 1799u);
+                            item = 0u; gen = true;
+                        }
+                        nextFrame += (uint32_t)__popcll(mTake);
+                    }
+                }
+#ifdef CRT_POOL_DENS
+                {
+                    const uint32_t gone = (uint32_t)__popcll(__builtin_amdgcn_ballot_w64(ended) & ~__builtin_amdgcn_ballot_w64(gen));
+                    if (gone) { const unsigned long long now = wall_clock64(); dens[44u + CRT_LIVE_BUCKET(live)] += (uint32_t)(now - liveClk); liveClk = now; live -= gone; }
+                }
+#endif
                 const kernarg_f cam = scene_floats(offsetof(Scene, camPos));
                 const f3 camPos = mk3(cam[0], cam[1], cam[2]);
                 f3 v = camPos;
@@ -434,6 +475,9 @@
                     seed = st[F_SEED * S + s]; meta = st[F_META * S + s]; obj = (int)(meta >> kMetaObjShift) - 1;
                 }
                 const bool mesh = act && obj >= 2;
+#ifdef CRT_POOL_DENS
+                dens[40u + CRT_LIVE_BUCKET(live)]++;
+#endif
                 CRT_DENS(14, 1); CRT_DENS(15, n); CRT_DENS_MASK(16, mesh);
                 rec4 s0 = {0, 0, 0, 0}, s1 = s0, s2 = s0, s3 = s0;
                 if (mesh) { const uint32_t so = sc.shadeOff + tri * 64u; s0 = ldg(geom, so); s1 = ldg(geom, so + 16u); s2 = ldg(geom, so + 32u); s3 = ldg(geom, so + 48u); cn.meshhits++; }
@@ -545,15 +589,16 @@
     if (lane == 0) for (int i = 0; i < 12; i++) atomicAdd(&g_poolStamps[i], pst[i]);
 #endif
 #ifdef CRT_POOL_DENS
-    if (lane == 0) for (int i = 0; i < 32; i++) if (dens[i]) atomicAdd(&g_poolDens[i], (unsigned long long)dens[i]);
+    dens[44u + CRT_LIVE_BUCKET(live)] += (uint32_t)(wall_clock64() - liveClk);
+    if (lane == 0) for (int i = 0; i < 48; i++) if (dens[i]) atomicAdd(&g_poolDens[i], (unsigned long long)dens[i]);
 #endif
 
 #ifdef CRT_POOL_TIMELINE
     if (lane == 0 && g_poolTimeline) { uint32_t hw; asm volatile("s_getreg_b32 %0, hwreg(HW_REG_HW_ID)" : "=s"(hw)); g_poolTimeline[3 * (size_t)blockIdx.x] = tl0; g_poolTimeline[3 * (size_t)blockIdx.x + 1] = wall_clock64(); g_poolTimeline[3 * (size_t)blockIdx.x + 2] = hw; }
 #endif
-    if (tileCost && lane == 0 && nStreams == (uint32_t)S) atomicMax(&tileCost[tl], (uint32_t)((wall_clock64() - clk0) * 64ull / (uint32_t)S));
+    if (tileCost && lane == 0 && nOwn == (uint32_t)S) atomicMax(&tileCost[tl], (uint32_t)((wall_clock64() - clk0) * 64ull / (uint32_t)S));
     if (launchClk && lane == 0) { const unsigned long long now = wall_clock64(), last = __hip_atomic_load(&launchClk[1], __ATOMIC_RELAXED, __HIP_MEMORY_SCOPE_AGENT), from = last > clk0 ? last : clk0; if (now > from) atomicAdd(&launchClk[2], now - from); }
-    if (COUNT && tileClocks && lane == 0 && groups == 1u) {
+    if (COUNT && tileClocks && lane == 0 && nOwn == frames) {
         tileClocks[2 * tl] = wall_clock64() - clk0;
         tileClocks[2 * tl + 1] = trips;
     }
@@ -575,7 +620,7 @@
 #ifndef CRT_POOL_EXTRA_LDS
 #define CRT_POOL_EXTRA_LDS 0
 #endif
-extern "C" uint32_t crt_pool_lds_bytes(uint32_t stackDepth, uint32_t streams) { return (stackDepth + 1u) * 64u * 2u + crt::F_COUNT * streams * 4u + 3u * 128u + (uint32_t)CRT_POOL_EXTRA_LDS; }
+extern "C" uint32_t crt_pool_lds_bytes(uint32_t stackDepth, uint32_t streams) { return (stackDepth + 1u) * 64u * 2u + crt::F_COUNT * streams * 4u + 3u * 128u + (streams > 64u ? 2u * streams : 0u) + (uint32_t)CRT_POOL_EXTRA_LDS; }
 extern "C" size_t crt_pool_scratch_bytes_per_window(uint32_t tileCount) { return (size_t)tileCount * 128u * 15u * 4u; }
 
 #ifdef CRT_POOL_STAMPS
@@ -589,8 +634,8 @@
 #ifdef CRT_POOL_DENS
 extern "C" int crt_debug_pool_density(unsigned long long* out, int reset)
 {
-    if (out && hipMemcpyFromSymbol(out, HIP_SYMBOL(crt::g_poolDens), 256) != hipSuccess) return -1;
-    if (reset) { unsigned long long z[32] = {}; if (hipMemcpyToSymbol(HIP_SYMBOL(crt::g_poolDens), z, 256) != hipSuccess) return -1; }
+    if (out && hipMemcpyFromSymbol(out, HIP_SYMBOL(crt::g_poolDens), 384) != hipSuccess) return -1;
+    if (reset) { unsigned long long z[48] = {}; if (hipMemcpyToSymbol(HIP_SYMBOL(crt::g_poolDens), z, 384) != hipSuccess) return -1; }
     return 0;
 }
 #endif
@@ -605,22 +650,27 @@
 #endif
 extern "C" hipError_t crt_launch_render_pool(const crt::Scene* sc, void* slab, void* facScratch, crt::Counters* counters, unsigned long long* tileClocks, const uint32_t* tileOrder,
                                              uint32_t tileFirst, uint32_t tileStride, uint32_t tileCount, uint32_t tilesX, uint32_t sppFirst,
-                                             uint32_t frames, uint32_t passes, int collectStats, uint32_t rankFirst, uint32_t* tileCost, unsigned long long* launchClk, hipStream_t stream)
+                                             uint32_t frames, uint32_t passes, int collectStats, uint32_t rankFirst, uint32_t waveFrames, const uint32_t* waveTab, uint32_t tabBlocks, uint32_t longFrames,
+                                             uint32_t* tileCost, unsigned long long* launchClk, hipStream_t stream)
 {
     if (tileCount == 0 || frames == 0) return hipSuccess;
     if (!sc->ref16ok) return hipErrorInvalidValue;
     const uint32_t S = crt_pool_streams(frames);
-    const uint32_t groups = (frames + S - 1u) / S;
-    if ((unsigned long long)tileCount * groups > 0x7fffffffull) return hipErrorInvalidValue;
+    const uint32_t wf = (S == 64u || waveFrames < S) ? S : waveFrames;
+    if (wf % S != 0u || wf > 0xff80u) return hipErrorInvalidValue;
+    if (S == 64u) waveTab = nullptr;
+    if (waveTab && (tabBlocks == 0u || longFrames == 0u || longFrames > frames)) return hipErrorInvalidValue;
+    const uint32_t groups = waveTab ? (frames - longFrames + S - 1u) / S : (frames + wf - 1u) / wf;
+    if ((unsigned long long)tileCount * ((frames + S - 1u) / S) > 0x7fffffffull) return hipErrorInvalidValue;
     if (rankFirst >= tileCount) return hipSuccess;
-    dim3 grid((tileCount - rankFirst) * groups), block(64);
+    dim3 grid(waveTab ? tabBlocks + (tileCount - rankFirst) * groups : (tileCount - rankFirst) * groups), block(64);
 #ifdef CRT_POOL_TIMELINE
     { static unsigned long long* buf = nullptr; static size_t cap = 0;
       if (cap < (size_t)grid.x) { if (buf) (void)hipFree(buf); (void)hipMalloc((void**)&buf, (size_t)grid.x * 24); cap = grid.x; (void)hipMemcpyToSymbol(HIP_SYMBOL(crt::g_poolTimeline), &buf, sizeof(buf)); }
       (void)hipMemsetAsync(buf, 0, (size_t)grid.x * 24, stream); g_timelineHost = buf; g_timelineCount = grid.x; }
 #endif
     const uint32_t ldsBytes = crt_pool_lds_bytes(sc->stackDepth, S);
-#define CRT_LAUNCH(K, C, SS) hipLaunchKernelGGL((crt::render_pool_kernel<K, C, SS>), grid, block, ldsBytes, stream, *sc, (float4*)slab, (float*)facScratch, counters, tileClocks, tileOrder, tileFirst, tileStride, tileCount, tilesX, sppFirst, frames, passes, groups, rankFirst, tileCost, launchClk)
+#define CRT_LAUNCH(K, C, SS) hipLaunchKernelGGL((crt::render_pool_kernel<K, C, SS>), grid, block, ldsBytes, stream, *sc, (float4*)slab, (float*)facScratch, counters, tileClocks, tileOrder, tileFirst, tileStride, tileCount, tilesX, sppFirst, frames, passes, groups, wf, waveTab, tabBlocks, longFrames, rankFirst, tileCost, launchClk)
 #define CRT_LAUNCH_S(K, C) do { if (S == 64u) CRT_LAUNCH(K, C, 64); else CRT_LAUNCH(K, C, CRT_POOL_STREAMS); } while (0)
     if (sc->kind == 0) { if (collectStats) CRT_LAUNCH_S(0, true); else CRT_LAUNCH_S(0, false); }
     else { if (collectStats) CRT_LAUNCH_S(1, true); else CRT_LAUNCH_S(1, false); }
```
